# LunaJang/Metabuli_work

Hardware: AMD Instinct MI355X
Metric: reads/sec classified (150bp & 10kb) vs GTDB-scale DB at 1/2/4/8 MI355X (higher is better)
Workload: dtype u64

## Files before the change

### metabuli_work_amd/classifier.py

```python
from __future__ import annotations

import ctypes
import dataclasses
import gzip
import os
from typing import Iterator, List, Optional, Tuple

import numpy as np

from . import _abi
from ._abi import KMER_DTYPE, MATCH_DTYPE, RESULT_DTYPE, TAXCNT_DTYPE, MtbParams, ptr
from ._lib import MtbError, check, lib


@dataclasses.dataclass
class LocalParameters:
    seqMode: int = 2
    kmerFormat: int = 1
    syncmer: int = 0
    smerLen: int = 5
    reducedAA: int = 0
    skipRedundancy: int = 0
    minScore: float = 0.0
    minSpScore: float = 0.0
# ... 106 lines not shown
        return self

    def __exit__(self, *a):
        self.close()

    @property
    def db_kmers(self) -> int:
        return int(lib().mtb_db_kmers(self.handle))

    @property
    def workspace_bytes(self) -> int:
        return int(lib().mtb_workspace_bytes(self.handle))

    OPEN_PHASES = ["read_s", "decode_s", "directory_s", "probe_lines_s", "run_index_s", "taxonomy_s", "total_s",
                   "records_alloc_s"]

    def open_phases(self) -> dict:
        out = (ctypes.c_double * len(self.OPEN_PHASES))()
        lib().mtb_open_phases(self.handle, out, len(self.OPEN_PHASES))
        return {k: round(float(v), 3) for k, v in zip(self.OPEN_PHASES, out)}

    def set_workspace_cap(self, nbytes: int) -> None:
        check(lib().mtb_set_workspace_cap(self.handle, int(nbytes)), "mtb_set_workspace_cap")

    def release_workspace(self) -> None:
        self._dev_batch = None
        check(lib().mtb_release_workspace(self.handle), "mtb_release_workspace")

    def set_stream(self, stream_ptr: int) -> None:
        check(lib().mtb_set_stream(self.handle, ctypes.c_void_p(stream_ptr)), "mtb_set_stream")

    def classify_batch(self, seq1: np.ndarray, off1: np.ndarray, seq2=None, off2=None, keep_stages: bool = False,
                       device_input: bool = False, fetch: bool = True, match_only: bool = False
                       ) -> Optional[BatchResult]:
        n = (len(off1) - 1) if not device_input else int(off1.numel()) - 1
        flags = (_abi.MTB_KEEP_STAGES if keep_stages else 0) | (_abi.MTB_INPUT_DEVICE if device_input else 0)
        if match_only:
            flags |= _abi.MTB_MATCH_ONLY
            fetch = False
        if device_input:
            _after_torch(seq1)
            ptrs = [ctypes.c_void_p(t.data_ptr()) if t is not None else ctypes.c_void_p(0)
                    for t in (seq1, off1, seq2, off2)]
        else:
            ptrs = [ptr(np.ascontiguousarray(a)) if a is not None else ctypes.c_void_p(0)
                    for a in (seq1, off1, seq2, off2)]
            self._keep = (seq1, off1, seq2, off2)
        res = np.zeros(n, RESULT_DTYPE) if fetch else None
        self._dev_batch = None
        rc = check(lib().mtb_classify_batch(self.handle, ptrs[0], ptrs[1], ptrs[2], ptrs[3], n, flags,
                                            ptr(res) if fetch else ctypes.c_void_p(0)), "mtb_classify_batch")
        if rc == _abi.MTB_RETRY:
            if keep_stages or match_only or n < 2:
                raise MtbError(f"mtb_classify_batch: {lib().mtb_last_error().decode()}")
            if not fetch:
                self._classify_halves_device(seq1, off1, seq2, off2, n, device_input)
                return None
            return self._classify_halves(seq1, off1, seq2, off2, n, device_input)
        if not fetch:
            return None
        return BatchResult(res, self.taxcnt(), *self.last_counts(), self.stage_ms())

    def _classify_halves_device(self, seq1, off1, seq2, off2, n, device_input) -> None:
        import torch

        dev = torch.device("cuda", self.device)
        mid = n // 2
        recs, pools, qk, mm = [], [], 0, 0
        stats, stage, kern = None, np.zeros(5, np.float32), np.zeros(7, np.float32)
        for lo, hi in ((0, mid), (mid, n)):
            o1 = off1[lo:hi + 1]
            o2 = off2[lo:hi + 1] if off2 is not None else None
            self.classify_batch(seq1, o1, seq2, o2, device_input=device_input, fetch=False)
            rec = torch.empty((hi - lo, _abi.RESULT_DTYPE.itemsize), dtype=torch.uint8, device=dev)
            self.copy_results(rec.data_ptr(), on_device=True)
            pool = torch.empty((max(self.n_taxcnt(), 1), _abi.TAXCNT_DTYPE.itemsize), dtype=torch.uint8, device=dev)
            nt = self.copy_taxcnt(pool.data_ptr(), on_device=True)
            q, m = self.last_counts()
            recs.append(rec)
            pools.append(pool[:nt])
            qk, mm = qk + q, mm + m
            st = self.stats()
            stats = st if stats is None else {k: (max(stats[k], v) if k == "max_read_matches" else
                                                  v if k in ("join_path", "uniform_units") else stats[k] + v)
                                              for k, v in st.items()}
            stage += self.stage_ms()
            kern += self.kernel_ms()
        recs[1].view(torch.int32).view(-1, _abi.RESULT_DTYPE.itemsize // 4)[:, 4] += pools[0].shape[0]
        torch.cuda.synchronize(dev)
        self._dev_batch = _DevBatch(torch.cat(recs), torch.cat(pools), qk, mm, stats, stage, kern)

    def _classify_halves(self, seq1, off1, seq2, off2, n, device_input) -> BatchResult:
        mid = n // 2
        parts = []
        for lo, hi in ((0, mid), (mid, n)):
            o1 = off1[lo:hi + 1]
            o2 = off2[lo:hi + 1] if off2 is not None else None
            parts.append(self.classify_batch(seq1, o1, seq2, o2, device_input=device_input))
        a, b = parts
        rb = b.results.copy()
        rb["taxcnt_offset"] += len(a.taxcnt)
        return BatchResult(np.concatenate([a.results, rb]), np.concatenate([a.taxcnt, b.taxcnt]),
                           a.query_kmers + b.query_kmers, a.matches + b.matches, a.stage_ms + b.stage_ms)

    def taxcnt(self) -> np.ndarray:
        if getattr(self, "_dev_batch", None) is not None:
            return self._dev_batch.taxcnt.cpu().numpy().reshape(-1).view(TAXCNT_DTYPE).copy()
        nt = ctypes.c_uint64(0)
        lib().mtb_get_taxcnt(self.handle, ctypes.c_void_p(0), 0, ctypes.byref(nt))
        tc = np.zeros(int(nt.value), TAXCNT_DTYPE)
        check(lib().mtb_get_taxcnt(self.handle, ptr(tc), len(tc), ctypes.byref(nt)), "mtb_get_taxcnt")
        return tc

    def last_counts(self) -> Tuple[int, int]:
        if getattr(self, "_dev_batch", None) is not None:
            return self._dev_batch.query_kmers, self._dev_batch.matches
        q, m = ctypes.c_uint64(0), ctypes.c_uint64(0)
        lib().mtb_last_counts(self.handle, ctypes.byref(q), ctypes.byref(m))
        return int(q.value), int(m.value)

    STATS = ["slots", "query_kmers", "matched_queries", "matches", "max_read_matches", "groups", "groups_ge2",
             "species_runs", "wave_runs", "wave_runs_emulated", "join_path", "live_matches", "gallop_queries",
             "spilled_matches", "long_run_queries", "filter_reruns", "db_records_read", "dup_aa_queries",
             "dup_key_queries", "uniform_units"]

    def stats(self) -> dict:
        if getattr(self, "_dev_batch", None) is not None:
            return dict(self._dev_batch.stats)
        out = (ctypes.c_uint64 * len(self.STATS))()
        lib().mtb_last_stats(self.handle, out, len(self.STATS))
        return {k: int(v) for k, v in zip(self.STATS, out)}

    def stage_ms(self) -> np.ndarray:
        if getattr(self, "_dev_batch", None) is not None:
            return self._dev_batch.stage_ms.copy()
        ms = (ctypes.c_float * 5)()
        lib().mtb_last_stage_ms(self.handle, ms, 5)
        return np.array(list(ms), np.float32)

    def kernel_ms(self) -> np.ndarray:
        if getattr(self, "_dev_batch", None) is not None:
            return self._dev_batch.kernel_ms.copy()
        ms = (ctypes.c_float * 7)()
        lib().mtb_last_kernel_ms(self.handle, ms, 7)
        return np.array(list(ms), np.float32)

    def _copy_dev(self, t, dst_ptr: int, on_device: bool) -> None:
        import torch

        del on_device
        if t.numel():
            torch.cuda.synchronize(t.device)
            check(lib().mtb_memcpy(ctypes.c_void_p(dst_ptr), ctypes.c_void_p(t.data_ptr()), t.numel()), "mtb_memcpy")

    def copy_results(self, dst_ptr: int, on_device: bool = True) -> None:
        if getattr(self, "_dev_batch", None) is not None:
            return self._copy_dev(self._dev_batch.results, dst_ptr, on_device)
        check(lib().mtb_copy_results(self.handle, ctypes.c_void_p(dst_ptr), int(on_device)), "mtb_copy_results")

    def n_taxcnt(self) -> int:
        if getattr(self, "_dev_batch", None) is not None:
            return int(self._dev_batch.taxcnt.shape[0])
        nt = ctypes.c_uint64(0)
        lib().mtb_get_taxcnt(self.handle, ctypes.c_void_p(0), 0, ctypes.byref(nt))
        return int(nt.value)

    def copy_taxcnt(self, dst_ptr: int, on_device: bool = True) -> int:
        if getattr(self, "_dev_batch", None) is not None:
            self._copy_dev(self._dev_batch.taxcnt, dst_ptr, on_device)
            return int(self._dev_batch.taxcnt.shape[0])
        nt = ctypes.c_uint64(0)
        check(lib().mtb_copy_taxcnt(self.handle, ctypes.c_void_p(dst_ptr), int(on_device), ctypes.byref(nt)),
              "mtb_copy_taxcnt")
        return int(nt.value)

    def query_kmers(self) -> np.ndarray:
        q = self.stats()["query_kmers"]
        out = np.zeros(q, KMER_DTYPE)
        nq = ctypes.c_uint64(0)
        check(lib().mtb_get_query_kmers(self.handle, ptr(out), q, ctypes.byref(nq)), "mtb_get_query_kmers")
        return out

    def matches(self) -> np.ndarray:
        _, m = self.last_counts()
        out = np.zeros(m, MATCH_DTYPE)
        nm = ctypes.c_uint64(0)
        check(lib().mtb_get_matches(self.handle, ptr(out), m, ctypes.byref(nm)), "mtb_get_matches")
        return out

    def assign_matches(self, matches: np.ndarray, query_len: np.ndarray) -> BatchResult:
        matches = np.ascontiguousarray(matches, MATCH_DTYPE)
        ql = np.ascontiguousarray(query_len, np.uint32)
        res = np.zeros(len(ql), RESULT_DTYPE)
        check(lib().mtb_assign_matches(self.handle, ptr(matches), len(matches), ptr(ql), len(ql), ptr(res)),
              "mtb_assign_matches")
        return BatchResult(res, self.taxcnt(), 0, len(matches), self.stage_ms())

    def copy_matches(self, matches=None, read_counts=None, query_len=None) -> None:
        arrs = [a for a in (matches, read_counts, query_len) if a is not None]
        on_dev = bool(arrs) and not isinstance(arrs[0], np.ndarray)

        def p(a):
            if a is None:
                return ctypes.c_void_p(0)
            return ctypes.c_void_p(a.data_ptr()) if on_dev else ptr(a)
        check(lib().mtb_copy_matches(self.handle, p(matches), p(read_counts), p(query_len), int(on_dev)),
              "mtb_copy_matches")
# ... 186 lines not shown
```

### metabuli_work_amd/csrc/mtb_api.hip

```cpp
#include <chrono>
#include <cmath>
#include <cstdio>
#include <cstring>
#include <string>
#include <vector>
#include <algorithm>
#include <memory>
#include <charconv>
#include <mutex>
#include <unordered_map>

#include "mtb_host.h"
#include "mtb_launch.h"
#include <cstdlib>

using namespace mtb;

#define HIP_TRY(x)                                                                                   \
    do {                                                                                             \
        hipError_t e_ = (x);                                                                         \
        if (e_ != hipSuccess) {                                                                      \
            set_error(std::string("HIP error ") + hipGetErrorString(e_) + " at " #x);                 \
            return e_ == hipErrorOutOfMemory ? MTB_ERR_OOM : MTB_ERR_HIP;                            \
        }                                                                                            \
// ... 80 lines not shown
    uint64_t D = 0;
    DbRec* db = nullptr;
    bool borrowedDb = false;
    std::shared_ptr<DbArrays> dbArrays;
    uint64_t* dirMem = nullptr;
    ProbeLine* lines = nullptr;
    uint64_t* lineP = nullptr;
    uint16_t* runOff = nullptr;
    ProbeExt* lineExt = nullptr;
    uint64_t* link = nullptr;
    AADir dir{};
    uint64_t rankLo = 0, rankHi = ~0ull;
    int joinMode = 0;
    uint64_t* tileRec = nullptr;
    uint32_t* tilePre = nullptr;
    uint64_t nTiles = 0;
    uint32_t sweepNom = 2048;
    uint32_t sweepLdsCap = ~0u;
    bool sweepSmall = false;
    bool filterThreadMajor = false;
    int sweepPersist = 1;
    uint32_t matchWinCap = ~0u;
    bool directJoin = true;
    bool directRetry = false;
    int pruneAfter = 2;
    int bigGroups = 1;
    bool fuseFilter = true;
    bool radixDigits = true;
    bool radixAtomicFirst = false;
    int binnedSort = 0;
    uint64_t binRcForce = 0;
    bool binDigits = true;
    bool uniformUnits = true;
    uint32_t upr = 0;
    uint64_t binHost[kSortBins] = {};
    bool noFilter = false;
    uint32_t spillShift = 0;
    bool sparse = false;
    uint32_t maxW = 0;
    uint32_t maxMate = 0;
    int sortLoFine = kQuerySortLoFine;
    bool forceGeneric = false;
    bool segsortGlobal = false;
    uint32_t mergeSeg = 0;
    int waveTaxon = -1;
    int emulateAll = 0;
    bool pruneCompact = true;
    bool noAlias = false;
    uint64_t aliasBytes = 0;
    int32_t* spOf = nullptr;
    int32_t maxTax = 0;
    int32_t *tNodeOf = nullptr, *tNodeTax = nullptr, *tParent = nullptr, *tDepth = nullptr, *tSpParent = nullptr;
    uint8_t* tFlags = nullptr;
    uint32_t cladePerMatch = 2;
    std::vector<int32_t> hNodeOf;
    std::vector<std::string> hRank;
    HostTaxonomy hTax;
    mutable std::vector<std::string> lineage;
    mutable std::once_flag lineageOnce;
    std::shared_ptr<void> pipelineCache;
    mutable mtb::TaxText taxText;
    mutable std::once_flag taxTextOnce;
    WsBudget ws;
    DevBuf seq1, off1, seq2, off2, meta, reserve, slotOff, qlen, scanTmp;
    DevBuf keysA, valsA, keysB, valsB, radixCounts, radixOffs;
    DevBuf readCnt, mOff, matches, matchesSorted, segScratch, maxSeg, errFlag;
    DevBuf ordKA, ordVA, ordKB, ordVB, matchWin, unitRead, unitInfo, mStage, mRank, mTotal, mDirect, ovFlag, waveList, waveCount, devStats;
    DevBuf qFrom, probeStats;
    DevBuf longList, longCnt;
    DevBuf qStart;
    uint32_t longCap = 0;
    DevBuf chunkIn, chunkCnt, chunkSrcOff;
    DevBuf liveCnt, liveOff;
    DevBuf runFlag, runCnt, runScan;
    DevBuf segLen;
    DevBuf sizeLists;
    DevBuf digA, digB;
    DevBuf binCnt, binTab;
    DevBuf maskOut1, maskOut2, maskProb, maskScale;
    DevBuf readLens;
    DevBuf readCnt64;
    uint64_t liveM = 0;
    double openS[8] = {0, 0, 0, 0, 0, 0, 0, 0};
    static constexpr int kNumStats = 20;
    uint64_t stats[kNumStats] = {};
    uint32_t chunkC = 1;
    uint64_t stageRegion = 0;
    uint64_t spillCap = 0;
    DevBuf emMap, emCnt, emScratch, emPacked, emCnt32, emOff;
    bool emValid = false;
    bool emPackedValid = false;
    std::vector<mtb_em_map> emHost;
    std::vector<uint32_t> spKmers;
    std::string dbDir;
    DevBuf local, paths, comb, conn, spScore, spKeep,
        pathCnt, gStart, sStart, runGroup, clade, tcPool, tcLen, tcOff, tcOut, results;
    uint32_t nReads = 0;
    uint64_t Q = 0, M = 0, nTaxcnt = 0;
    uint64_t Qall = 0;
    double presentShare = 0.5;
    const uint64_t* qKeys = nullptr;
    const uint32_t* qSlots = nullptr;
    bool keepStages = false;
    bool probed = false;
    bool matchOnly = false;
    float stageMs[5] = {0, 0, 0, 0, 0};
    hipEvent_t ev[6]{};
    static constexpr int kNumKern = 7;
    float kernMs[kNumKern] = {0, 0, 0, 0, 0, 0, 0};
    hipEvent_t kev[2 * kNumKern]{};
};

static std::vector<DevBuf*> batch_bufs(mtb_ctx* c);

static void bind_workspace(mtb_ctx* c, size_t cap) {
    c->ws.cap = cap;
    if (const char* e = getenv("MTB_WORKSPACE_CAP")) {
        char* end = nullptr;
        double v = strtod(e, &end);
        const char u = end ? *end : 0;
        v *= u == 'G' || u == 'g' ? 1e9 : u == 'M' || u == 'm' ? 1e6 : u == 'K' || u == 'k' ? 1e3 : 1.0;
        c->ws.cap = v > 0 ? (size_t)v : 0;
    }
    for (DevBuf* b : batch_bufs(c)) b->budget = &c->ws;
}

static void free_db(mtb_ctx* c) {
    if (c->dbArrays) {
        c->dbArrays.reset();
        c->db = nullptr;
        c->dirMem = nullptr;
        c->lines = nullptr;
        c->lineP = nullptr;
        c->runOff = nullptr;
        c->lineExt = nullptr;
        c->link = nullptr;
        return;
    }
    if (c->borrowedDb) c->db = nullptr;
    void* ptrs[] = {c->db, c->dirMem, c->lines, c->lineP, c->runOff, c->lineExt, c->link, c->spOf, c->tNodeOf, c->tNodeTax, c->tParent, c->tDepth, c->tSpParent, c->tFlags};
    for (void* p : ptrs)
        if (p) hipFree(p);
    c->db = nullptr;
    c->dirMem = nullptr;
    c->lines = nullptr;
    c->lineP = nullptr;
    c->runOff = nullptr;
    c->lineExt = nullptr;
    c->link = nullptr;
}

template <typename T>
static hipError_t upload(T** dst, const std::vector<T>& v, hipStream_t s) {
    hipError_t e = hipMalloc((void**)dst, std::max<size_t>(1, v.size()) * sizeof(T));
    if (e != hipSuccess) return e;
    if (!v.empty()) e = hipMemcpyAsync(*dst, v.data(), v.size() * sizeof(T), hipMemcpyHostToDevice, s);
    return e;
}

static int validate_params(const mtb_params* p) {
    if (p->reduced_aa) { set_error("reduced-AA DBs (ReducedKmerMatcher) are out of scope"); return MTB_ERR_UNSUPPORTED; }
    if (p->em && p->db_parts > 1) { set_error("--em needs the whole DB in one context"); return MTB_ERR_UNSUPPORTED; }
    if (p->mask_mode && !(p->mask_prob > 0.0f && p->mask_prob <= 1.0f)) { set_error("mask_prob must be in (0, 1]"); return MTB_ERR_ARG; }
    if (p->kmer_format != 1 && p->kmer_format != 2) { set_error("kmer_format must be 1 or 2"); return MTB_ERR_UNSUPPORTED; }
    if (p->syncmer && p->kmer_format != 2) { set_error("syncmer requires kmer_format 2"); return MTB_ERR_UNSUPPORTED; }
    if (p->syncmer && (p->smer_len < 1 || p->smer_len > 8)) { set_error("smer_len must be in [1, 8]"); return MTB_ERR_ARG; }
    if (p->seq_mode < 1 || p->seq_mode > 3) { set_error("seq_mode must be 1, 2 or 3"); return MTB_ERR_ARG; }
// ... 385 lines not shown

#define MTB_BATCH_BUFS(X) \
    X(seq1) X(off1) X(seq2) X(off2) X(meta) X(reserve) X(slotOff) X(qlen) X(scanTmp) X(keysA) X(valsA) X(keysB) \
    X(valsB) X(radixCounts) X(radixOffs) X(readCnt) X(mOff) X(matches) X(matchesSorted) X(segScratch) X(maxSeg) \
    X(errFlag) X(ordKA) X(ordVA) X(ordKB) X(ordVB) X(matchWin) X(unitRead) X(unitInfo) X(waveList) X(waveCount) \
    X(devStats) X(mStage) X(mRank) X(mDirect) X(ovFlag) X(mTotal) X(qFrom) X(probeStats) X(longList) X(longCnt) \
    X(qStart) X(chunkIn) X(chunkCnt) X(chunkSrcOff) X(liveCnt) X(liveOff) X(segLen) X(sizeLists) X(digA) \
    X(digB) X(binCnt) X(binTab) X(local) X(paths) X(comb) X(conn) X(spScore) X(spKeep) X(runFlag) X(runCnt) \
    X(runScan) X(pathCnt) X(gStart) X(sStart) X(runGroup) X(clade) X(tcPool) X(tcLen) X(tcOff) X(tcOut) X(results) \
    X(emMap) X(emCnt) X(emScratch) X(emPacked) X(emCnt32) X(emOff) X(maskOut1) X(maskOut2) X(maskProb) \
    X(maskScale) X(readLens) X(readCnt64)
static std::vector<DevBuf*> batch_bufs(mtb_ctx* c) {
#define MTB_BUF_PTR(n) &c->n,
    return {MTB_BATCH_BUFS(MTB_BUF_PTR)};
#undef MTB_BUF_PTR
}

static const char* const* batch_buf_names() {
#define MTB_BUF_NAME(n) #n,
    static const char* const names[] = {MTB_BATCH_BUFS(MTB_BUF_NAME)};
#undef MTB_BUF_NAME
    return names;
}

void mtb_close(mtb_ctx* c) {
    if (!c) return;
    hipSetDevice(c->device);
    if (c->stream) hipStreamSynchronize(c->stream);
    free_db(c);
    if (c->tileRec) hipFree(c->tileRec);
    if (c->tilePre) hipFree(c->tilePre);
    c->pipelineCache.reset();
    hipSetDevice(c->device);
    for (DevBuf* b : batch_bufs(c)) b->release();
    for (auto& e : c->ev)
        if (e) hipEventDestroy(e);
    for (auto& e : c->kev)
        if (e) hipEventDestroy(e);
    if (c->ownStream && c->stream) hipStreamDestroy(c->stream);
    delete c;
}

int mtb_set_stream(mtb_ctx* c, void* stream) {
    if (!c) return MTB_ERR_ARG;
    if (c->ownStream && c->stream) hipStreamDestroy(c->stream);
    if (stream) {
        c->stream = (hipStream_t)stream;
        c->ownStream = false;
    } else {
        HIP_TRY(hipStreamCreateWithFlags(&c->stream, hipStreamNonBlocking));
        c->ownStream = true;
    }
    return MTB_OK;
}

uint64_t mtb_db_kmers(const mtb_ctx* c) { return c ? c->D : 0; }

uint64_t mtb_workspace_bytes(const mtb_ctx* c) { return c ? c->ws.used : 0; }

int mtb_open_phases(const mtb_ctx* c, double* sec, int n) {
    if (!c || !sec) return MTB_ERR_ARG;
    for (int i = 0; i < n && i < 8; i++) sec[i] = c->openS[i];
    return MTB_OK;
}

int mtb_set_workspace_cap(mtb_ctx* c, uint64_t bytes) {
    if (!c) return MTB_ERR_ARG;
    c->ws.cap = bytes;
    return MTB_OK;
}

int mtb_release_workspace(mtb_ctx* c) {
    if (!c) return MTB_ERR_ARG;
    mtb::ctx_release_workspace(c);
    void* p = nullptr;
    if (hipMalloc(&p, 64u << 20) == hipSuccess) hipFree(p);
    return hipDeviceSynchronize() == hipSuccess ? MTB_OK : MTB_ERR_HIP;
}

int mtb_ctx_device(const mtb_ctx* c) { return c ? c->device : 0; }

}

static AssignArgs assign_args(const mtb_params& p) {
    AssignArgs a;
    a.em = p.em ? 1 : 0;
    a.kmerFormat = p.kmer_format;
    if (p.syncmer) {
        a.dnaShift = (8 - p.smer_len) * 3;
        a.maxCodonShift = 8 - p.smer_len;
    } else {
        a.dnaShift = 3;
        a.maxCodonShift = 1;
    }
    a.denominator = (p.seq_mode == 1 || p.seq_mode == 2) ? 100 : 1000;
    a.minConsCnt = p.min_cons_cnt;
    a.minConsCntEuk = p.min_cons_cnt_euk;
    a.accessionLevel = p.accession_level;
    a.minScore = p.min_score;
    a.minSpScore = p.min_sp_score;
    a.tieRatio = p.tie_ratio;
    a.generic = 0;
    return a;
}

static int assign_stage(mtb_ctx* c, uint32_t n, bool keep) {
    hipStream_t s = c->stream;
    HIP_TRY(c->errFlag.ensure(sizeof(int)));
    const uint64_t M = c->M;
    AssignArgs a = assign_args(c->par);
    a.generic = c->forceGeneric ? 1 : 0;
    a.waveTaxon = c->waveTaxon;
    a.bigGroups = c->bigGroups;
    a.emulateAll = c->emulateAll;
    if (a.dnaShift <= 0) { set_error("syncmer smer_len 8 gives a zero dnaShift"); return MTB_ERR_ARG; }
    HIP_TRY(c->readCnt.ensure(sizeof(uint32_t) * (n + 1)));
    const uint64_t Mc = std::max<uint64_t>(M, 1);
    HIP_TRY(c->results.ensure(sizeof(mtb_result) * std::max<uint32_t>(n, 1)));
    HIP_TRY(c->matchesSorted.ensure(sizeof(mtb_match) * Mc));
    HIP_TRY(c->maxSeg.ensure(sizeof(uint32_t)));
    launch_max_seg(c->mOff.as<uint64_t>(), n, c->maxSeg.as<uint32_t>(), s);
    uint32_t maxSeg = 0;
    HIP_TRY(hipMemcpyAsync(&maxSeg, c->maxSeg.p, sizeof(uint32_t), hipMemcpyDeviceToHost, s));
    HIP_TRY(hipStreamSynchronize(s));
    const bool prune = !keep && !c->forceGeneric;
    if (maxSeg > kSegSortLds || c->forceGeneric || c->segsortGlobal || (c->mergeSeg && maxSeg > c->mergeSeg))
        HIP_TRY(c->segScratch.ensure(6 * sizeof(uint64_t) * Mc));
    const bool compact = prune && maxSeg > kSegSortRegs && !c->segsortGlobal && c->pruneCompact;
    if (compact) HIP_TRY(c->segLen.ensure(sizeof(uint32_t) * (n + 1)));
    if (maxSeg > 128) HIP_TRY(c->sizeLists.ensure(sizeof(uint32_t) * (4 * (size_t)n + 4)));
    c->keepStages = !prune;
    HIP_TRY(c->liveCnt.ensure(sizeof(uint32_t) * (n + 1)));
    HIP_TRY(c->liveOff.ensure(sizeof(uint64_t) * (n + 1)));
    HIP_TRY(c->scanTmp.ensure(sizeof(uint64_t) * scan_tmp_elems(n + 1)));
    HIP_TRY(hipEventRecord(c->kev[10], s));
    if (c->sparse && (!prune || (maxSeg > kSegSortSparse && !compact) || c->segsortGlobal ||
                      (c->mergeSeg && maxSeg > c->mergeSeg))) {
        launch_compact_segments(c->mDirect.as<SegMatch>(), c->slotOff.as<uint64_t>(), c->chunkC,
                                c->mOff.as<uint64_t>(), n, c->matches.as<mtb_match>(), c->spillShift, s,
                                c->stats[13] ? 2 : 0);
        c->sparse = false;
    }
    HIP_TRY(launch_segsort(c->matches.as<mtb_match>(), c->mOff.as<uint64_t>(), n, Mc, c->matchesSorted.as<mtb_match>(),
                           c->segScratch.as<uint64_t>(), maxSeg, c->forceGeneric || c->segsortGlobal,
                           prune ? c->liveCnt.as<uint32_t>() : nullptr, c->mergeSeg,
                           prune_min_matches(a.minConsCnt, a.minConsCntEuk, a.maxCodonShift), s,
                           c->sparse ? c->mDirect.as<SegMatch>() : nullptr, c->slotOff.as<uint64_t>(),
                           c->chunkC | c->spillShift << 16,
                           compact ? c->segLen.as<uint32_t>() : nullptr,
                           c->maxSeg.as<uint32_t>(), c->pruneAfter, maxSeg > 128 ? c->sizeLists.as<uint32_t>() : nullptr));
    c->sparse = false;
    const mtb_match* kIn = c->matchesSorted.as<mtb_match>();
    const uint64_t* kOff = c->mOff.as<uint64_t>();
    uint64_t kM = M;
    HIP_TRY(c->runCnt.ensure(sizeof(uint32_t) * 2 * ((size_t)n + 1)));
    HIP_TRY(c->runScan.ensure(sizeof(uint64_t) * 2 * ((size_t)n + 1)));
    uint32_t* grpCnt = c->runCnt.as<uint32_t>();
    uint32_t* runCnt = grpCnt + n + 1;
    if (prune) {
        exclusive_scan_u32(c->liveCnt.as<uint32_t>(), n, c->liveOff.as<uint64_t>(), c->scanTmp.p, s);
        HIP_TRY(hipMemcpyAsync(&kM, c->liveOff.as<uint64_t>() + n, sizeof(uint64_t), hipMemcpyDeviceToHost, s));
        HIP_TRY(hipStreamSynchronize(s));
        if (kM > M) { set_error("internal error: K5 kept more matches than it sorted"); return MTB_ERR_INTERNAL; }
        HIP_TRY(c->runFlag.ensure(std::max<uint64_t>(kM, 1)));
        launch_run_flags(c->matchesSorted.as<mtb_match>(), c->mOff.as<uint64_t>(), c->liveOff.as<uint64_t>(), n,
                         c->matches.as<mtb_match>(), c->runFlag.as<uint8_t>(), grpCnt, runCnt, c->errFlag.as<int>(),
                         s);
        kIn = c->matches.as<mtb_match>();
        kOff = c->liveOff.as<uint64_t>();
    } else {
        HIP_TRY(c->runFlag.ensure(Mc));
        launch_run_flags(kIn, kOff, kOff, n, nullptr, c->runFlag.as<uint8_t>(), grpCnt, runCnt, c->errFlag.as<int>(), s);
    }
    c->liveM = kM;
    c->stats[11] = kM;
    const uint64_t Kc = std::max<uint64_t>(kM, 1);
    const uint64_t Mn = std::max<uint64_t>(Kc, n);
    std::vector<std::pair<char*, size_t>> dead;
    if (!c->noAlias) {
        std::vector<DevBuf*> d = {&c->mDirect, &c->segScratch, &c->mStage, &c->mRank, &c->matchWin, &c->chunkIn};
        if (prune) {
            for (DevBuf* b : {&c->matchesSorted, &c->keysA, &c->valsA, &c->keysB, &c->valsB}) d.push_back(b);
        } else {
            d.push_back(&c->matches);
        }
        for (DevBuf* b : d)
            if (b->p && b->bytes >= (1u << 20)) dead.push_back({b->as<char>(), b->bytes});
        std::sort(dead.begin(), dead.end(), [](auto& a, auto& b) { return a.second > b.second; });
    }
    struct Need {
        DevBuf* own;
        uint64_t bytes;
        void* p;
    };
    Need need[] = {{&c->local, path_bytes() * Kc, nullptr},
                   {&c->paths, path_bytes() * Kc, nullptr},
                   {&c->comb, path_bytes() * Kc, nullptr},
                   {&c->conn, Kc, nullptr},
                   {&c->spScore, sizeof(float) * Kc, nullptr},
                   {&c->spKeep, Kc, nullptr},
                   {&c->waveList, sizeof(uint64_t) * Kc, nullptr},
                   {&c->pathCnt, sizeof(uint32_t) * (Kc + 1), nullptr},
                   {&c->gStart, sizeof(uint64_t) * (Kc + 1), nullptr},
                   {&c->sStart, sizeof(uint64_t) * (Kc + 1), nullptr},
                   {&c->runGroup, sizeof(uint64_t) * (Kc + 1), nullptr},
                   {&c->clade, clade_bytes() * Kc * c->cladePerMatch, nullptr},
                   {&c->tcPool, sizeof(mtb_taxcnt) * Kc, nullptr},
                   {&c->ordKA, sizeof(uint64_t) * (Mn + 1), nullptr},
                   {&c->ordVA, sizeof(uint64_t) * (Mn + 1), nullptr},
                   {&c->ordKB, sizeof(uint64_t) * (Mn + 1), nullptr},
                   {&c->ordVB, sizeof(uint64_t) * (Mn + 1), nullptr}};
    std::vector<Need*> order;
    for (Need& x : need) order.push_back(&x);
    std::stable_sort(order.begin(), order.end(), [](Need* a, Need* b) { return a->bytes > b->bytes; });
    c->aliasBytes = 0;
    for (Need* x : order) {
        const size_t b = (x->bytes + 255) & ~(size_t)255;
        for (auto& r : dead)
            if (r.second >= b) {
                x->p = r.first;
                r.first += b;
                r.second -= b;
                c->aliasBytes += b;
                break;
            }
        if (!x->p) {
            HIP_TRY(x->own->ensure(x->bytes));
            x->p = x->own->p;
        }
    }
    HIP_TRY(c->waveCount.ensure(sizeof(uint32_t)));
    HIP_TRY(hipEventRecord(c->kev[11], s));
    HIP_TRY(hipEventRecord(c->kev[12], s));
    HIP_TRY(c->radixCounts.ensure(sizeof(uint32_t) * radix_counts_elems(Mn + 1)));
    HIP_TRY(c->radixOffs.ensure(sizeof(uint64_t) * (radix_counts_elems(Mn + 1) + 1)));
    HIP_TRY(c->scanTmp.ensure(sizeof(uint64_t) * scan_tmp_elems(radix_counts_elems(Mn + 1) + n + Mn + 2)));
    TaxDevice t{c->tNodeOf, c->tNodeTax, c->tParent, c->tDepth, c->tFlags, c->tSpParent, c->maxTax};
    AssignScratch sc{need[0].p,
                     need[1].p,
                     need[2].p,
                     (uint8_t*)need[3].p,
                     (uint32_t*)need[7].p,
                     (uint64_t*)need[8].p,
                     (uint64_t*)need[9].p,
                     (uint64_t*)need[10].p,
                     c->runFlag.as<uint8_t>(),
                     grpCnt,
                     runCnt,
                     c->runScan.as<uint64_t>(),
                     c->runScan.as<uint64_t>() + n + 1,
                     (float*)need[4].p,
                     (uint64_t*)need[6].p,
                     c->waveCount.as<uint32_t>(),
                     (uint8_t*)need[5].p,
                     c->scanTmp.p,
                     (uint64_t*)need[13].p,
                     (uint64_t*)need[14].p,
                     (uint64_t*)need[15].p,
                     (uint64_t*)need[16].p,
                     c->radixCounts.as<uint32_t>(),
                     c->radixOffs.as<uint64_t>(),
                     need[11].p,
                     c->cladePerMatch};
    mtb_taxcnt* tcPool = (mtb_taxcnt*)need[12].p;
    c->stats[3] = M;
    c->stats[4] = maxSeg;
    launch_assign(kIn, kOff, c->qlen.as<uint32_t>(), n, kM, a, t, sc, tcPool,
                  c->results.as<mtb_result>(), c->devStats.as<unsigned long long>(), c->stats + 5, s);
    HIP_TRY(hipEventRecord(c->kev[13], s));
    HIP_TRY(c->tcLen.ensure(sizeof(uint32_t) * (n + 1)));
    HIP_TRY(c->tcOff.ensure(sizeof(uint64_t) * (n + 1)));
    launch_taxcnt_len(c->results.as<mtb_result>(), n, c->tcLen.as<uint32_t>(), s);
    exclusive_scan_u32(c->tcLen.as<uint32_t>(), n, c->tcOff.as<uint64_t>(), c->scanTmp.p, s);
    uint64_t NT = 0;
    HIP_TRY(hipMemcpyAsync(&NT, c->tcOff.as<uint64_t>() + n, sizeof(uint64_t), hipMemcpyDeviceToHost, s));
    HIP_TRY(hipStreamSynchronize(s));
    HIP_TRY(c->tcOut.ensure(sizeof(mtb_taxcnt) * std::max<uint64_t>(NT, 1)));
    launch_compact_taxcnt(tcPool, kOff, c->results.as<mtb_result>(), c->tcOff.as<uint64_t>(), n,
                          c->tcOut.as<mtb_taxcnt>(), s);
    c->nTaxcnt = NT;
    c->emValid = false;
    c->emPackedValid = false;
    if (c->par.em) {
        const uint64_t nS = std::max<uint64_t>(c->stats[7], 1);
        HIP_TRY(c->emScratch.ensure(8 * nS));
        HIP_TRY(c->emMap.ensure(8 * (uint64_t)kEmTop * std::max<uint32_t>(n, 1)));
        HIP_TRY(c->emCnt.ensure(std::max<uint32_t>(n, 1)));
        launch_em_top(kIn, kOff, n, sc, c->results.as<mtb_result>(), c->emScratch.p, c->emMap.p,
                      c->emCnt.as<uint8_t>(), s);
        HIP_TRY(hipGetLastError());
        c->emValid = true;
    }
    return MTB_OK;
}

static int join_stage(mtb_ctx* c, const uint8_t* dSeq1, const uint64_t* dOff1, const uint8_t* dSeq2,
                      const uint64_t* dOff2, uint32_t n, uint64_t U, uint32_t C, uint64_t R, uint64_t Rc) {
    hipStream_t s = c->stream;
    const bool probe = c->probed;
    const bool filt = c->lines && (!c->noFilter || probe);
    const bool fused = filt && !probe && c->fuseFilter;
    if (!fused) {
        HIP_TRY(c->keysA.ensure(8 * Rc));
        HIP_TRY(c->valsA.ensure(4 * Rc));
        HIP_TRY(c->keysB.ensure(8 * Rc));
        HIP_TRY(c->valsB.ensure(4 * Rc));
    }
    HIP_TRY(c->radixCounts.ensure(sizeof(uint32_t) * radix_counts_elems(Rc)));
    HIP_TRY(c->radixOffs.ensure(sizeof(uint64_t) * (radix_counts_elems(Rc) + 1)));
    HIP_TRY(c->scanTmp.ensure(sizeof(uint64_t) * scan_tmp_elems(radix_counts_elems(Rc) + n + 1)));
    HIP_TRY(c->mTotal.ensure(sizeof(unsigned long long) * kStageRegions));
    HIP_TRY(c->probeStats.ensure(sizeof(unsigned long long) * kProbeStatsLen));
    HIP_TRY(hipMemsetAsync(c->probeStats.p, 0, sizeof(unsigned long long) * kProbeStatsLen, s));
    HIP_TRY(hipEventRecord(c->kev[0], s));
    if (!fused)
        launch_extract(dSeq1, dOff1, dSeq2, dOff2, c->meta.as<ReadMeta>(), c->slotOff.as<uint64_t>(),
                       c->unitRead.as<uint32_t>(), U, C, c->tables, c->par.kmer_format, c->par.syncmer,
                       c->par.smer_len, c->keysA.as<uint64_t>(), c->unitInfo.as<uint64_t>(), s, c->upr);
    HIP_TRY(hipEventRecord(c->kev[1], s));
    uint64_t Q = R;
    const uint64_t* qk = c->keysA.as<uint64_t>();
    const uint32_t* qi = nullptr;
    const uint64_t* qf = nullptr;
    HIP_TRY(hipEventRecord(c->kev[2], s));
    const bool digits = fused && c->radixDigits && c->sortLoFine == kQuerySortLo;
    uint64_t binRc = 0;
    if (fused) {
        uint64_t cap = std::min<uint64_t>(R, (uint64_t)((double)R * c->presentShare) + 4096);
        bool binned = digits && c->binnedSort && (c->binnedSort == 2 || cap >= (1ull << 22));
        for (int pass = 0; pass < 2 && binned; pass++) {
            uint64_t rc = c->binRcForce ? c->binRcForce : (cap + cap / 16) / kSortBins + 256;
            rc = (rc + 63) / 64 * 64;
            const uint64_t slots = rc * kSortBins;
            HIP_TRY(c->keysB.ensure(8 * slots));
            HIP_TRY(c->valsB.ensure(4 * slots));
            HIP_TRY(c->digA.ensure(slots));
            HIP_TRY(c->binCnt.ensure(sizeof(unsigned long long) * kSortBins));
            Q = launch_extract_filter(dSeq1, dOff1, dSeq2, dOff2, c->meta.as<ReadMeta>(), c->slotOff.as<uint64_t>(),
                                      c->unitRead.as<uint32_t>(), U, C, c->tables, c->par.kmer_format, c->par.syncmer,
                                      c->par.smer_len, c->unitInfo.as<uint64_t>(), c->lines, c->keysB.as<uint64_t>(),
                                      c->valsB.as<uint32_t>(), c->mTotal.as<unsigned long long>(), c->rankLo,
                                      c->rankHi, &c->Qall, slots, false, s,
                                      c->binDigits ? c->digA.as<uint8_t>() : nullptr,
                                      c->binCnt.as<unsigned long long>(), rc, c->binHost, c->upr);
            HIP_TRY(hipGetLastError());
            if (R) c->presentShare = std::max(c->presentShare, std::min(1.0, 1.125 * (double)Q / (double)R));
            bool over = false;
            for (int r = 0; r < kSortBins; r++) over |= c->binHost[r] > rc;
            if (!over) {
                binRc = rc;
                break;
// ... 216 lines not shown
                    c->mRank.ensure(sizeof(uint32_t) * want) == hipSuccess) {
                    c->spillCap = want;
                    HIP_TRY(hipMemsetAsync(c->probeStats.p, 0, sizeof(unsigned long long) * kProbeStatsLen, s));
                    continue;
                }
                (void)hipGetLastError();
            }
            nSpill = 0;
            direct = false;
            if (sweep && !unstaged_join(c->lines != nullptr, c->D, Q, std::min<uint32_t>(c->matchWinCap, 3072)))
                launch_match_windows(qk, Q, c->db, c->D, c->dir, c->par.kmer_format, c->matchWin.as<uint64_t>(), s);
            HIP_TRY(c->mStage.ensure(sizeof(mtb_match) * c->stageRegion * kStageRegions));
            HIP_TRY(c->mRank.ensure(sizeof(uint32_t) * c->stageRegion * kStageRegions));
            HIP_TRY(hipMemsetAsync(c->probeStats.p, 0, sizeof(unsigned long long) * kProbeStatsLen, s));
            continue;
        }
        M = 0;
        uint64_t most = 0;
        for (unsigned long long t : regTot) {
            M += t;
            most = std::max<uint64_t>(most, t);
        }
        if (most <= c->stageRegion || M >= kMaxBatchMatches) break;
        c->stageRegion = most + most / 8;
        HIP_TRY(c->mStage.ensure(sizeof(mtb_match) * c->stageRegion * kStageRegions));
        HIP_TRY(c->mRank.ensure(sizeof(uint32_t) * c->stageRegion * kStageRegions));
        HIP_TRY(hipMemsetAsync(c->probeStats.p, 0, sizeof(unsigned long long) * kProbeStatsLen, s));
    }
    if (cnt64) launch_cnt64_counts(cnt64, n, c->readCnt.as<uint32_t>(), s);
    HIP_TRY(hipEventRecord(c->kev[7], s));
    exclusive_scan_u32(c->readCnt.as<uint32_t>(), n, c->mOff.as<uint64_t>(), c->scanTmp.p, s);
    if (direct) {
        HIP_TRY(hipMemcpyAsync(&M, c->mOff.as<uint64_t>() + n, sizeof(uint64_t), hipMemcpyDeviceToHost, s));
        HIP_TRY(hipStreamSynchronize(s));
    }
    if (M >= kMaxBatchMatches) {
        set_error("batch produced >= 2^32 matches: split it into smaller batches");
        return MTB_ERR_ARG;
    }
    c->M = M;
    HIP_TRY(c->matches.ensure(sizeof(mtb_match) * std::max<uint64_t>(M, 1)));
    HIP_TRY(hipEventRecord(c->kev[8], s));
    c->stats[13] = nSpill;
    c->sparse = direct && !c->keepStages && !c->forceGeneric && !c->matchOnly;
    if (c->sparse && nSpill) {
        launch_compact_segments(c->mDirect.as<SegMatch>(), c->slotOff.as<uint64_t>(), C, c->mOff.as<uint64_t>(), n,
                                c->matches.as<mtb_match>(), c->spillShift, s, 1);
        launch_spill_scatter(c->mStage.as<mtb_match>(), c->mRank.as<uint32_t>(), c->mTotal.as<unsigned long long>(),
                             nSpill, c->mOff.as<uint64_t>(), n, c->matches.as<mtb_match>(), c->errFlag.as<int>(), s);
    } else if (direct && !c->sparse) {
        launch_compact_segments(c->mDirect.as<SegMatch>(), c->slotOff.as<uint64_t>(), C, c->mOff.as<uint64_t>(), n,
                                c->matches.as<mtb_match>(), c->spillShift, s);
        launch_spill_scatter(c->mStage.as<mtb_match>(), c->mRank.as<uint32_t>(), c->mTotal.as<unsigned long long>(),
                             nSpill, c->mOff.as<uint64_t>(), n, c->matches.as<mtb_match>(), c->errFlag.as<int>(), s);
    } else if (!direct)
        launch_match_transpose(c->mStage.as<mtb_match>(), c->mRank.as<uint32_t>(), c->stageRegion,
                               c->mTotal.as<unsigned long long>(), c->mOff.as<uint64_t>(), n,
                               c->matches.as<mtb_match>(), c->errFlag.as<int>(), s);
    HIP_TRY(hipEventRecord(c->kev[9], s));
    HIP_TRY(hipEventRecord(c->ev[3], s));
    return MTB_OK;
}

static int batch_error(int err) {
    switch (err) {
        case kErrTaxid:
            set_error("a selected reference k-mer has taxID 0 or no species in taxID_list (KmerMatcher.cpp:432-441)");
            return MTB_ERR_DB;
        case kErrProbeStash:
            set_error("a DB AA run holds >= 2^24 k-mers (probe join stash limit): use MTB_JOIN=sort");
            return MTB_ERR_DB;
        case kErrStagedRead:
            set_error("internal error: a staged or spilled match names a read outside the batch or past its segment");
            return MTB_ERR_INTERNAL;
        case kErrProbeCount:
            set_error("internal error: emitted matches disagree with the probe counts");
            return MTB_ERR_INTERNAL;
        case kErrRunOutsideDb:
            set_error("internal error: K4 found an AA run starting past the DB's end (run index or probe lines "
                      "inconsistent with the DB records)");
            return MTB_ERR_INTERNAL;
        case kErrLiveCount:
            set_error("internal error: K5 kept more live matches than a read's segment holds");
            return MTB_ERR_INTERNAL;
        default:
            set_error("internal error: device error flag " + std::to_string(err));
            return MTB_ERR_INTERNAL;
    }
}

static int check_err_flag(mtb_ctx* c) {
    int err = 0;
    HIP_TRY(hipMemcpy(&err, c->errFlag.p, sizeof(int), hipMemcpyDeviceToHost));
    return err ? batch_error(err) : MTB_OK;
}

static int mask_mates(mtb_ctx* c, const uint8_t* seq1, const uint64_t* off1, const uint8_t* seq2, const uint64_t* off2,
                      uint32_t n, const uint8_t** out1, const uint8_t** out2) {
    hipStream_t s = c->stream;
    uint64_t nb[2] = {0, 0};
    HIP_TRY(hipMemcpyAsync(&nb[0], off1 + n, sizeof(uint64_t), hipMemcpyDeviceToHost, s));
    if (seq2) HIP_TRY(hipMemcpyAsync(&nb[1], off2 + n, sizeof(uint64_t), hipMemcpyDeviceToHost, s));
    HIP_TRY(hipStreamSynchronize(s));
    const uint64_t most = std::max(nb[0], nb[1]);
    HIP_TRY(c->maskProb.ensure(sizeof(float) * (most + 1)));
    HIP_TRY(c->maskScale.ensure(sizeof(double) * tantan_scale_elems(most, n)));
    const TantanTables tt = make_tantan_tables(c->par.mask_prob);
    HIP_TRY(c->maskOut1.ensure(nb[0] + 1));
    launch_tantan_mask(seq1, off1, n, tt, c->maskProb.as<float>(), c->maskScale.as<double>(), c->maskOut1.as<uint8_t>(), s);
    *out1 = c->maskOut1.as<uint8_t>();
    if (seq2) {
        HIP_TRY(c->maskOut2.ensure(nb[1] + 1));
        launch_tantan_mask(seq2, off2, n, tt, c->maskProb.as<float>(), c->maskScale.as<double>(),
                           c->maskOut2.as<uint8_t>(), s);
        *out2 = c->maskOut2.as<uint8_t>();
    }
    HIP_TRY(hipGetLastError());
    return MTB_OK;
}

extern "C" {

int mtb_memcpy(void* dst, const void* src, uint64_t bytes) {
    if (bytes && (!dst || !src)) { set_error("null argument"); return MTB_ERR_ARG; }
    if (bytes) HIP_TRY(hipMemcpy(dst, src, bytes, hipMemcpyDefault));
    return MTB_OK;
}

int mtb_line_ext_check(mtb_ctx* c, uint64_t* out) {
    if (!c || !out) return MTB_ERR_ARG;
    out[0] = out[1] = out[2] = 0;
    if (!c->lineExt || !c->runOff) { set_error("no run-length lines (MTB_LINE_EXT=0, or no run index)"); return MTB_ERR_ARG; }
    HIP_TRY(hipSetDevice(c->device));
    DevBuf cnt;
    HIP_TRY(cnt.ensure(3 * sizeof(unsigned long long)));
    HIP_TRY(hipMemsetAsync(cnt.p, 0, 3 * sizeof(unsigned long long), c->stream));
    launch_line_ext_check(c->lines, c->lineP, c->runOff, c->lineExt, cnt.as<unsigned long long>(), c->stream);
    HIP_TRY(hipGetLastError());
    HIP_TRY(hipMemcpyAsync(out, cnt.p, 3 * sizeof(uint64_t), hipMemcpyDeviceToHost, c->stream));
    HIP_TRY(hipStreamSynchronize(c->stream));
    if (out[2]) {
        set_error("internal error: " + std::to_string(out[2]) + " runs from the run-length lines disagree with the run index");
        return MTB_ERR_INTERNAL;
    }
    return MTB_OK;
}

int mtb_link_check(mtb_ctx* c, uint64_t* out) {
    if (!c || !out) return MTB_ERR_ARG;
    out[0] = out[1] = out[2] = 0;
    if (!c->link || !c->lines) { set_error("no link lines (MTB_LINK_LINES=0, the probe or sweep join, or no memory for them)"); return MTB_ERR_ARG; }
    HIP_TRY(hipSetDevice(c->device));
    DevBuf cnt;
    HIP_TRY(cnt.ensure(3 * sizeof(unsigned long long)));
    HIP_TRY(hipMemsetAsync(cnt.p, 0, 3 * sizeof(unsigned long long), c->stream));
    launch_link_check(c->lines, c->link, cnt.as<unsigned long long>(), c->stream);
    HIP_TRY(hipGetLastError());
    HIP_TRY(hipMemcpyAsync(out, cnt.p, 3 * sizeof(uint64_t), hipMemcpyDeviceToHost, c->stream));
    HIP_TRY(hipStreamSynchronize(c->stream));
    if (out[2]) {
        set_error("internal error: " + std::to_string(out[2]) + " link-line bits disagree with the probe lines");
        return MTB_ERR_INTERNAL;
    }
    return MTB_OK;
}

// ... 915 lines not shown
```

### metabuli_work_amd/csrc/mtb_assign.hip

```cpp
#include <algorithm>
#include <vector>

#include "mtb_launch.h"
#include "mtb_stdsort.h"

namespace mtb {

struct Path {
    int start, end;
    float score;
    int hd, depth;
    uint32_t sm, em;
};

__device__ __forceinline__ void match_key(const mtb_match& m, uint64_t& hi, uint64_t& lo) {
    hi = ((uint64_t)m.species_id << 32) | ((uint64_t)info_frame(m.qinfo) << 29) | (info_pos(m.qinfo) & 0x1FFFFFFFu);
    lo = ((uint64_t)m.hamming << 56) | ((uint64_t)(m.dna_encoding & 0xFFFFFFu) << 32) | m.target_id;
}

__device__ __forceinline__ bool key_gt(uint64_t ah, uint64_t al, uint64_t bh, uint64_t bl) {
    return ah > bh || (ah == bh && al > bl);
}

constexpr int kSmallSeg = 512;
static_assert(kSmallSeg == (int)kSegSortRegs, "one register-sort bound");
constexpr int kBlockSeg = 8192;
constexpr uint32_t kSegSkip = 0xFFFFFFFFu;

__device__ __forceinline__ long seg_len(const uint64_t* __restrict__ mOff, const uint32_t* __restrict__ segLen,
                                        uint32_t r) {
    if (!segLen) return (long)(mOff[r + 1] - mOff[r]);
    const uint32_t v = segLen[r];
    return v == kSegSkip ? -1 : (long)v;
}

template <int K, int J, int E, typename F>
__device__ __forceinline__ void bitonic_stages(F& f) {
    f(std::integral_constant<int, K>{}, std::integral_constant<int, J>{});
    if constexpr (J > 1) bitonic_stages<K, J / 2, E>(f);
    else if constexpr (K < 64 * E) bitonic_stages<K * 2, K, E>(f);
}

template <int J>
__device__ __forceinline__ uint64_t xor_lane64c(uint64_t v, int lane) {
    return (uint64_t)xor_lane<J>((uint32_t)(v >> 32), lane) << 32 | xor_lane<J>((uint32_t)v, lane);
}

template <int E>
__device__ __forceinline__ void wave_bitonic_sort(uint64_t (&h)[E], uint64_t (&l)[E], uint32_t (&x)[E], int lane) {
    auto stage = [&](auto kc, auto jc) {
        constexpr int k = decltype(kc)::value, j = decltype(jc)::value;
        if constexpr (j >= 64) {
            constexpr int js = j >> 6;
#pragma unroll
            for (int sl = 0; sl < E; sl++) {
                if (sl & js) continue;
                const int s2 = sl | js;
                const bool up = ((64 * sl + lane) & k) == 0;
                if (key_gt(h[sl], l[sl], h[s2], l[s2]) == up) {
                    const uint64_t th = h[sl], tl = l[sl];
                    const uint32_t tx = x[sl];
                    h[sl] = h[s2]; l[sl] = l[s2]; x[sl] = x[s2];
                    h[s2] = th; l[s2] = tl; x[s2] = tx;
                }
            }
        } else {
            const bool lower = (lane & j) == 0;
#pragma unroll
            for (int sl = 0; sl < E; sl++) {
                const bool up = ((64 * sl + lane) & k) == 0;
                const uint64_t ph = xor_lane64c<j>(h[sl], lane), pl = xor_lane64c<j>(l[sl], lane);
                const uint32_t px = xor_lane<j>(x[sl], lane);
                const bool takeP = (key_gt(h[sl], l[sl], ph, pl) == (lower == up));
                if (takeP) { h[sl] = ph; l[sl] = pl; x[sl] = px; }
            }
        }
    };
    bitonic_stages<2, 1, E>(stage);
}

struct MatchIn {
    const mtb_match* __restrict__ p;
    uint64_t base;
    __device__ __forceinline__ mtb_match full(uint32_t e) const { return p[base + e]; }
};
struct SegIn {
    const SegMatch* __restrict__ p;
    uint64_t base;
    uint64_t seqBits;
    __device__ __forceinline__ mtb_match full(uint32_t e) const { return seg_expand(p[base + e], seqBits); }
};

__device__ __forceinline__ bool sparse_read(const SegMatch* seg, const uint64_t* __restrict__ inOff, uint32_t inCS,
                                            uint32_t r, long n) {
    if (!seg) return false;
    const uint64_t cap = ((inOff[r + 1] - inOff[r]) * (inCS & 0xFFFFu)) >> (inCS >> 16);
    return (uint64_t)n <= cap;
}
__device__ __forceinline__ SegIn sparse_in(const SegMatch* seg, const uint64_t* __restrict__ inOff, uint32_t inCS,
                                           uint32_t r) {
    return SegIn{seg, inOff[r] * (inCS & 0xFFFFu), (uint64_t)(r + 1) << 32};
}

template <typename K>
__device__ __forceinline__ uint32_t lds_insert(K* tab, uint32_t tn, K key) {
    uint32_t i = (uint32_t)(((uint64_t)key * 0x9E3779B97F4A7C15ull) >> 40) & (tn - 1);
    while (true) {
        const K prev = atomicCAS(&tab[i], (K)0, key);
        if (prev == 0 || prev == key) return i;
        i = (i + 1) & (tn - 1);
    }
}

template <int E2>
__device__ __forceinline__ void sort_live(mtb_match* __restrict__ out, uint64_t seqBits,
                                          uint64_t base, int nLive, int lane, const uint64_t* cH,
                                          const uint64_t* cL, const uint32_t* cX) {
    uint64_t h[E2], l[E2];
    uint32_t x[E2];
#pragma unroll
    for (int sl = 0; sl < E2; sl++) {
        const int e = 64 * sl + lane;
        const bool v = e < nLive;
        h[sl] = v ? cH[e] : ~0ull;
        l[sl] = v ? cL[e] : ~0ull;
        x[sl] = v ? cX[e] : 0u;
    }
    wave_bitonic_sort<E2>(h, l, x, lane);
#pragma unroll
    for (int sl = 0; sl < E2; sl++) {
        const int e = 64 * sl + lane;
        if (e < nLive) {
            mtb_match m;
            m.qinfo = ((h[sl] >> 29) & 7ull) << 61 | seqBits | (uint32_t)(h[sl] & 0x1FFFFFFFu);
            m.target_id = (uint32_t)l[sl];
            m.species_id = (uint32_t)(h[sl] >> 32);
            m.dna_encoding = (uint32_t)(l[sl] >> 32) & 0xFFFFFFu;
            m.right_end_hamming = (uint16_t)(x[sl] >> 16);
            m.hamming = (uint8_t)(l[sl] >> 56);
            m.pad = 0;
            out[base + e] = m;
        }
    }
}

template <int E>
struct PruneLds {
    union {
        struct {
            uint32_t spKey[128 * E];
            uint32_t pairKey[128 * E];
            uint32_t pairCnt[128 * E];
        } t;
        struct {
            uint64_t cH[64 * E], cL[64 * E];
            uint32_t cX[64 * E];
        } c;
    };
};
template <int E>
__device__ __forceinline__ PruneLds<E>& prune_lds() {
    __shared__ PruneLds<E> lds;
    return lds;
}
template <int E>
__device__ __forceinline__ uint8_t* run_live_lds() {
    __shared__ uint8_t runLive[64 * E];
    return runLive;
}

template <int E, typename In>
__device__ __forceinline__ void prune_then_sort(const In& in, mtb_match* __restrict__ out, uint64_t base, int n, int lane,
                                                uint32_t* __restrict__ liveCnt, uint32_t r, uint32_t pm) {
    constexpr uint32_t T = 128 * E;
    constexpr uint32_t kLive = 0x80000000u;
    PruneLds<E>& L = prune_lds<E>();
    uint32_t *spKey = L.t.spKey, *pairKey = L.t.pairKey, *pairCnt = L.t.pairCnt;
    for (uint32_t i = lane; i < T; i += 64) {
        spKey[i] = 0;
        pairKey[i] = 0;
        pairCnt[i] = 0;
    }
    __syncthreads();
    uint64_t h[E], l[E];
    uint32_t ps[E], ss[E], rx[E];
#pragma unroll
    for (int sl = 0; sl < E; sl++) {
        const int e = 64 * sl + lane;
        h[sl] = l[sl] = 0;
        ps[sl] = ss[sl] = rx[sl] = 0;
        if (e < n) {
            const mtb_match m = in.full((uint32_t)e);
            match_key(m, h[sl], l[sl]);
            rx[sl] = (uint32_t)m.right_end_hamming << 16;
            ss[sl] = lds_insert<uint32_t>(spKey, T, (uint32_t)(h[sl] >> 32));
            ps[sl] = lds_insert<uint32_t>(pairKey, T, (ss[sl] << 3 | ((uint32_t)(h[sl] >> 29) & 7u)) + 1u);
            atomicAdd(&pairCnt[ps[sl]], 1u);
        }
    }
    __syncthreads();
#pragma unroll
    for (int sl = 0; sl < E; sl++)
        if (64 * sl + lane < n && pairCnt[ps[sl]] >= pm) spKey[ss[sl]] |= kLive;
    __syncthreads();
    bool live[E];
#pragma unroll
    for (int sl = 0; sl < E; sl++) live[sl] = 64 * sl + lane < n && (spKey[ss[sl]] & kLive);
    __syncthreads();
    uint64_t *cH = L.c.cH, *cL = L.c.cL;
    uint32_t* cX = L.c.cX;
    const uint64_t lt = (1ull << lane) - 1;
    int nLive = 0;
#pragma unroll
    for (int sl = 0; sl < E; sl++) {
        const uint64_t m = __ballot(live[sl]);
        if (live[sl]) {
            const int p = nLive + (int)__popcll(m & lt);
            cH[p] = h[sl];
            cL[p] = l[sl];
            cX[p] = rx[sl] | (uint32_t)(64 * sl + lane);
        }
        nLive += (int)__popcll(m);
    }
    __syncthreads();
    const uint64_t seqBits = nLive ? in.full(0).qinfo & (0x1FFFFFFFull << 32) : 0;
    if (nLive <= 64) sort_live<1>(out, seqBits, base, nLive, lane, cH, cL, cX);
    else if (E >= 2 && nLive <= 128) sort_live<(E >= 2 ? 2 : 1)>(out, seqBits, base, nLive, lane, cH, cL, cX);
    else if (E >= 4 && nLive <= 256) sort_live<(E >= 4 ? 4 : 1)>(out, seqBits, base, nLive, lane, cH, cL, cX);
    else sort_live<E>(out, seqBits, base, nLive, lane, cH, cL, cX);
    if (lane == 0) liveCnt[r] = (uint32_t)nLive;
}

template <int E, typename K>
__device__ __forceinline__ void wave_bitonic_keys(K (&k)[E], int lane) {
    auto stage = [&](auto kc, auto jc) {
        constexpr int kk = decltype(kc)::value, j = decltype(jc)::value;
        if constexpr (j >= 64) {
            constexpr int js = j >> 6;
#pragma unroll
            for (int sl = 0; sl < E; sl++) {
                if (sl & js) continue;
                const int s2 = sl | js;
                const bool up = ((64 * sl + lane) & kk) == 0;
                if ((k[sl] > k[s2]) == up) {
                    const K t = k[sl];
                    k[sl] = k[s2];
                    k[s2] = t;
                }
            }
        } else {
            const bool lower = (lane & j) == 0;
#pragma unroll
            for (int sl = 0; sl < E; sl++) {
                const bool up = ((64 * sl + lane) & kk) == 0;
                K pk;
                if constexpr (sizeof(K) == 8) pk = (K)xor_lane64c<j>((uint64_t)k[sl], lane);
                else pk = (K)xor_lane<j>((uint32_t)k[sl], lane);
                if ((k[sl] > pk) == (lower == up)) k[sl] = pk;
            }
        }
    };
    bitonic_stages<2, 1, E>(stage);
}

template <int ES, typename K>
__device__ __forceinline__ void lds_sort_keys(K* a, int n, int lane) {
    K k[ES];
#pragma unroll
    for (int sl = 0; sl < ES; sl++) {
        const int e = 64 * sl + lane;
        k[sl] = e < n ? a[e] : (K)~(K)0;
    }
    wave_bitonic_keys<ES, K>(k, lane);
#pragma unroll
    for (int sl = 0; sl < ES; sl++) {
        const int e = 64 * sl + lane;
        if (e < n) a[e] = k[sl];
    }
}

template <int E, typename K>
__device__ __forceinline__ void lds_sort_keys_n(K* a, int n, int lane) {
    if (n <= 64) lds_sort_keys<1, K>(a, n, lane);
    else if (E >= 2 && n <= 128) lds_sort_keys<(E >= 2 ? 2 : 1), K>(a, n, lane);
    else if (E >= 4 && n <= 256) lds_sort_keys<(E >= 4 ? 4 : 1), K>(a, n, lane);
    else lds_sort_keys<E, K>(a, n, lane);
}

template <int E>
struct RankLds {
    union {
        struct {
            uint32_t spKey[128 * E];
            uint32_t pairKey[128 * E];
            uint32_t pairCnt[128 * E];
        } t;
        struct {
            uint64_t key[64 * E];
            uint64_t lo[64 * E];
            uint32_t sp[64 * E];
            uint32_t rx[64 * E];
        } c;
    };
};

template <int E>
__device__ __forceinline__ RankLds<E>& rank_lds() {
    __shared__ RankLds<E> lds;
    return lds;
}

template <int E, typename In>
__device__ __forceinline__ void prune_rank_sort(const In& in, mtb_match* __restrict__ out, uint64_t base, int n, int lane,
                                                uint32_t* __restrict__ liveCnt, uint32_t r, uint32_t pm) {
    constexpr uint32_t T = 128 * E;
    constexpr uint32_t kLive = 0x80000000u;
    RankLds<E>& L = rank_lds<E>();
    uint32_t *spKey = L.t.spKey, *pairKey = L.t.pairKey, *pairCnt = L.t.pairCnt;
    for (uint32_t i = lane; i < T; i += 64) {
        spKey[i] = 0;
        pairKey[i] = 0;
        pairCnt[i] = 0;
    }
    __syncthreads();
    uint64_t h[E], l[E];
    uint32_t ps[E], ss[E], rx[E];
#pragma unroll
    for (int sl = 0; sl < E; sl++) {
        const int e = 64 * sl + lane;
        h[sl] = l[sl] = 0;
        ps[sl] = ss[sl] = rx[sl] = 0;
        if (e < n) {
            const mtb_match m = in.full((uint32_t)e);
            match_key(m, h[sl], l[sl]);
            rx[sl] = (uint32_t)m.right_end_hamming << 16;
            ss[sl] = lds_insert<uint32_t>(spKey, T, (uint32_t)(h[sl] >> 32));
            ps[sl] = lds_insert<uint32_t>(pairKey, T, (ss[sl] << 3 | ((uint32_t)(h[sl] >> 29) & 7u)) + 1u);
            atomicAdd(&pairCnt[ps[sl]], 1u);
        }
    }
    __syncthreads();
#pragma unroll
    for (int sl = 0; sl < E; sl++)
        if (64 * sl + lane < n && pairCnt[ps[sl]] >= pm) spKey[ss[sl]] |= kLive;
    __syncthreads();
    bool live[E];
#pragma unroll
    for (int sl = 0; sl < E; sl++) live[sl] = 64 * sl + lane < n && (spKey[ss[sl]] & kLive);
    uint32_t wide = 0;
#pragma unroll
    for (int sl = 0; sl < E; sl++) wide |= (uint32_t)(h[sl] >> 56) | ((uint32_t)(h[sl] >> 28) & 1u);
    const bool direct = __ballot(wide != 0) == 0;
    const uint64_t lt = (1ull << lane) - 1;
    if (!direct) {
        uint32_t* spList = pairCnt;
        int S = 0;
        for (uint32_t i0 = 0; i0 < T; i0 += 64) {
            const uint32_t v = spKey[i0 + lane];
            const bool lv = (v & kLive) != 0;
            const uint64_t m = __ballot(lv);
            if (lv) spList[S + (int)__popcll(m & lt)] = v & ~kLive;
            S += (int)__popcll(m);
        }
        __syncthreads();
        lds_sort_keys_n<E, uint32_t>(spList, S, lane);
        __syncthreads();
        for (int e = lane; e < S; e += 64) {
            const uint32_t v = spList[e];
            uint32_t i = (uint32_t)(((uint64_t)v * 0x9E3779B97F4A7C15ull) >> 40) & (T - 1);
            while ((spKey[i] & ~kLive) != v) i = (i + 1) & (T - 1);
            pairKey[i] = (uint32_t)e;
        }
        __syncthreads();
    }
    const int frameAt = direct ? 37 : 38;
    uint64_t key[E];
    int nLive = 0;
#pragma unroll
    for (int sl = 0; sl < E; sl++) {
        const uint64_t m = __ballot(live[sl]);
        const uint32_t p = (uint32_t)(nLive + (int)__popcll(m & lt));
        if (direct)
            key[sl] = live[sl] ? ((h[sl] >> 29) << 37 | (h[sl] & 0x0FFFFFFFull) << 9 | p) : 0;
        else
            key[sl] = live[sl] ? ((uint64_t)pairKey[ss[sl]] << 41 | ((h[sl] >> 29) & 7ull) << 38 |
                                  (h[sl] & 0x1FFFFFFFull) << 9 | p)
                               : 0;
        nLive += (int)__popcll(m);
    }
    __syncthreads();
#pragma unroll
    for (int sl = 0; sl < E; sl++)
        if (live[sl]) {
            const uint32_t p = (uint32_t)(key[sl] & 511u);
            L.c.key[p] = key[sl];
            L.c.lo[p] = l[sl];
            L.c.sp[p] = (uint32_t)(h[sl] >> 32);
            L.c.rx[p] = rx[sl];
        }
    __syncthreads();
    lds_sort_keys_n<E, uint64_t>(L.c.key, nLive, lane);
    __syncthreads();
    const uint64_t seqBits = nLive ? in.full(0).qinfo & (0x1FFFFFFFull << 32) : 0;
    for (int e = lane; e < nLive; e += 64) {
        const uint64_t k = L.c.key[e];
        const uint32_t p = (uint32_t)(k & 511u);
        const uint64_t pre = k >> 9, lo = L.c.lo[p];
        int at = e;
        for (int j = e - 1; j >= 0 && (L.c.key[j] >> 9) == pre; j--) at -= L.c.lo[L.c.key[j] & 511u] > lo;
        for (int j = e + 1; j < nLive && (L.c.key[j] >> 9) == pre; j++) at += L.c.lo[L.c.key[j] & 511u] < lo;
        mtb_match m;
        m.qinfo = ((k >> frameAt) & 7ull) << 61 | seqBits | (uint32_t)((k >> 9) & ((1ull << (frameAt - 9)) - 1));
        m.target_id = (uint32_t)lo;
        m.species_id = L.c.sp[p];
        m.dna_encoding = (uint32_t)(lo >> 32) & 0xFFFFFFu;
        m.right_end_hamming = (uint16_t)(L.c.rx[p] >> 16);
        m.hamming = (uint8_t)(lo >> 56);
        m.pad = 0;
        out[base + at] = m;
    }
    if (lane == 0) liveCnt[r] = (uint32_t)nLive;
}

template <int E, typename In>
__device__ __forceinline__ void sort_then_prune(const In& in, mtb_match* __restrict__ out, uint64_t base, int n,
                                                int lane, uint32_t* __restrict__ liveCnt, uint32_t r, uint32_t pm) {
    uint64_t h[E], l[E];
    uint32_t x[E];
#pragma unroll
    for (int sl = 0; sl < E; sl++) {
        const int e = 64 * sl + lane;
        h[sl] = ~0ull;
        l[sl] = ~0ull;
        x[sl] = 0;
        if (e < n) {
            const mtb_match m = in.full((uint32_t)e);
            match_key(m, h[sl], l[sl]);
            x[sl] = (uint32_t)m.right_end_hamming << 16;
        }
    }
    const uint64_t seqBits = in.full(0).qinfo & (0x1FFFFFFFull << 32);
    wave_bitonic_sort<E>(h, l, x, lane);
    uint8_t* runLive = run_live_lds<E>();
    const uint64_t lt = (1ull << lane) - 1;
    const int far = lane + (int)pm - 1;
    uint32_t rid[E];
    bool pair[E];
    uint32_t runs = 0;
    uint64_t prevLast = ~0ull;
#pragma unroll
    for (int sl = 0; sl < E; sl++) {
        const int e = 64 * sl + lane;
        const uint64_t sf = h[sl] >> 29;
        const uint64_t a = __shfl(sf, far & 63, 64);
        const uint64_t b = __shfl(h[sl + 1 < E ? sl + 1 : sl] >> 29, far & 63, 64);
        uint64_t pv = __shfl_up(sf, 1, 64);
        if (lane == 0) pv = prevLast;
        prevLast = __shfl(sf, 63, 64);
        pair[sl] = e + (int)pm - 1 < n && (far < 64 ? a : b) == sf;
        const bool start = e < n && (e == 0 || (pv >> 3) != (sf >> 3));
        const uint64_t m = __ballot(start);
        rid[sl] = runs + (uint32_t)__popcll(m & lt) + (uint32_t)start - 1u;
        runs += (uint32_t)__popcll(m);
        runLive[64 * sl + lane] = 0;
    }
    __syncthreads();
#pragma unroll
    for (int sl = 0; sl < E; sl++)
        if (pair[sl]) runLive[rid[sl]] = 1;
    __syncthreads();
    uint32_t kept = 0;
#pragma unroll
    for (int sl = 0; sl < E; sl++) {
        const int e = 64 * sl + lane;
        const bool live = e < n && runLive[rid[sl]];
        const uint64_t m = __ballot(live);
        if (live) {
            mtb_match o;
            o.qinfo = ((h[sl] >> 29) & 7ull) << 61 | seqBits | (uint32_t)(h[sl] & 0x1FFFFFFFu);
            o.target_id = (uint32_t)l[sl];
            o.species_id = (uint32_t)(h[sl] >> 32);
            o.dna_encoding = (uint32_t)(l[sl] >> 32) & 0xFFFFFFu;
            o.right_end_hamming = (uint16_t)(x[sl] >> 16);
            o.hamming = (uint8_t)(l[sl] >> 56);
            o.pad = 0;
            out[base + kept + (uint32_t)__popcll(m & lt)] = o;
        }
        kept += (uint32_t)__popcll(m);
    }
    if (lane == 0) liveCnt[r] = kept;
}

template <int E, typename In, int kMode = 2>
__device__ __forceinline__ void segsort_regs(const In& in, mtb_match* __restrict__ out, uint64_t base, int n, int lane,
                                             uint32_t* __restrict__ liveCnt, uint32_t r, uint32_t pm) {
    if constexpr (E >= 2 && kMode == 2) {
        if (liveCnt) {
            prune_rank_sort<E>(in, out, base, n, lane, liveCnt, r, pm);
            return;
        }
        if constexpr (E > 2) return;
    } else if constexpr (E >= 2 && kMode == 1) {
        if (liveCnt && pm <= 64) {
            sort_then_prune<E>(in, out, base, n, lane, liveCnt, r, pm);
            return;
        }
    } else if constexpr (E >= 2 && kMode == 0) {
        if (liveCnt) {
            prune_then_sort<E>(in, out, base, n, lane, liveCnt, r, pm);
            return;
        }
        if constexpr (E > 2) return;
    }
    uint64_t h[E], l[E];
    uint32_t x[E];
#pragma unroll
    for (int sl = 0; sl < E; sl++) {
        const int e = 64 * sl + lane;
        h[sl] = ~0ull;
        l[sl] = ~0ull;
        x[sl] = (uint32_t)e;
        if (e < n) match_key(in.full((uint32_t)e), h[sl], l[sl]);
    }
    wave_bitonic_sort<E>(h, l, x, lane);
    if (!liveCnt) {
#pragma unroll
        for (int sl = 0; sl < E; sl++) {
            const int e = 64 * sl + lane;
            if (e < n) out[base + e] = in.full(x[sl]);
        }
        return;
    }
    if constexpr (E == 1) {
    uint8_t* runLive = run_live_lds<E>();
    const uint64_t lt = (1ull << lane) - 1;
    bool pair[E];
    uint32_t rid[E];
    uint32_t runs = 0;
#pragma unroll
    for (int sl = 0; sl < E; sl++) {
        const int e = 64 * sl + lane;
        const uint64_t sf = h[sl] >> 29;
        const uint64_t far = __shfl(sf, min(lane + (int)pm - 1, 63), 64);
        uint64_t pv = __shfl_up(sf, 1, 64);
        if (lane == 0) pv = ~0ull;
        pair[sl] = e + (int)pm - 1 < n && far == sf;
        const bool start = e < n && (e == 0 || (pv >> 3) != (sf >> 3));
        const uint64_t m = __ballot(start);
        rid[sl] = runs + (uint32_t)__popcll(m & lt) + (uint32_t)start - 1u;
        runs += (uint32_t)__popcll(m);
        runLive[64 * sl + lane] = 0;
    }
    __syncthreads();
#pragma unroll
    for (int sl = 0; sl < E; sl++)
        if (pair[sl]) runLive[rid[sl]] = 1;
    __syncthreads();
    uint32_t kept = 0;
#pragma unroll
    for (int sl = 0; sl < E; sl++) {
        const int e = 64 * sl + lane;
        const bool live = e < n && runLive[rid[sl]];
        const uint64_t m = __ballot(live);
        if (live) out[base + kept + (uint32_t)__popcll(m & lt)] = in.full(x[sl]);
        kept += (uint32_t)__popcll(m);
    }
    if (lane == 0) liveCnt[r] = kept;
    }
}

template <typename In>
__device__ __forceinline__ void segsort_small_run(const In& in, mtb_match* __restrict__ out, uint64_t base, int n,
                                                  int lane, uint32_t* __restrict__ liveCnt, uint32_t r, uint32_t pm) {
    if (n <= 1 || (liveCnt && n < (int)pm)) {
        if (lane == 0 && n == 1 && !liveCnt) out[base] = in.full(0);
        if (lane == 0 && liveCnt) liveCnt[r] = 0;
        return;
    }
    if (n <= 64) segsort_regs<1>(in, out, base, n, lane, liveCnt, r, pm);
    else segsort_regs<2>(in, out, base, n, lane, liveCnt, r, pm);
}

__global__ void __launch_bounds__(64) k_segsort_small(const mtb_match* __restrict__ in, const uint64_t* __restrict__ mOff,
                                                      const SegMatch* __restrict__ seg,
                                                      const uint64_t* __restrict__ inOff, uint32_t inC,
                                                      uint32_t nReads, mtb_match* __restrict__ out,
                                                      uint32_t* __restrict__ liveCnt, uint32_t pm,
                                                      const uint32_t* __restrict__ segLen) {
    const uint32_t r = blockIdx.x;
    if (r >= nReads) return;
    const uint64_t base = mOff[r];
    const long nl = seg_len(mOff, segLen, r);
    if (nl < 0 || nl > 128) return;
    const int n = (int)nl;
    if (sparse_read(seg, inOff, inC, r, n)) segsort_small_run(sparse_in(seg, inOff, inC, r), out, base, n, threadIdx.x, liveCnt, r, pm);
    else segsort_small_run(MatchIn{in, base}, out, base, n, threadIdx.x, liveCnt, r, pm);
}

template <int E, int kMode>
__global__ void __launch_bounds__(64) k_segsort_regs(const mtb_match* __restrict__ in, const uint64_t* __restrict__ mOff,
                                                     const SegMatch* __restrict__ seg,
                                                     const uint64_t* __restrict__ inOff, uint32_t inC,
                                                     uint32_t nReads, mtb_match* __restrict__ out,
                                                     uint32_t* __restrict__ liveCnt, uint32_t pm,
                                                     const uint32_t* __restrict__ segLen,
                                                     const uint32_t* __restrict__ list) {
    const uint32_t r = list ? list[blockIdx.x] : blockIdx.x;
    if (r >= nReads) return;
    const uint64_t base = mOff[r];
    const long nl = seg_len(mOff, segLen, r);
    if (nl <= 32 * E || nl > 64 * E) return;
    const int n = (int)nl;
    if (sparse_read(seg, inOff, inC, r, n))
        segsort_regs<E, SegIn, kMode>(sparse_in(seg, inOff, inC, r), out, base, n,
                                       (int)threadIdx.x, liveCnt, r, pm);
    else
        segsort_regs<E, MatchIn, kMode>(MatchIn{in, base}, out, base, n, (int)threadIdx.x, liveCnt, r, pm);
}

template <int kThreads, typename Idx>
__device__ void block_bitonic(uint64_t* H, uint64_t* Lo, Idx* I, long p2) {
    for (long k = 2; k <= p2; k <<= 1)
        for (long j = k >> 1; j > 0; j >>= 1) {
            for (long t = threadIdx.x; t < (p2 >> 1); t += kThreads) {
                const long i = ((t & ~(j - 1)) << 1) | (t & (j - 1));
                const long ixj = i + j;
                const bool up = (i & k) == 0;
                const uint64_t ah = H[i], al = Lo[i], bh = H[ixj], bl = Lo[ixj];
                if (key_gt(ah, al, bh, bl) == up) {
                    H[i] = bh; Lo[i] = bl; H[ixj] = ah; Lo[ixj] = al;
                    const Idx x = I[i]; I[i] = I[ixj]; I[ixj] = x;
                }
            }
            __threadfence_block();
            __syncthreads();
        }
}

template <int kThreads>
__device__ uint32_t block_scan_u32(uint32_t x, uint32_t* total, uint32_t* sWave) {
    constexpr int kW = kThreads / 64;
    const int lane = threadIdx.x & 63, w = threadIdx.x >> 6;
    uint32_t inc = x;
#pragma unroll
    for (int d = 1; d < 64; d <<= 1) {
        const uint32_t y = __shfl_up(inc, d, 64);
        if (lane >= d) inc += y;
    }
    if (lane == 63) sWave[w] = inc;
    __syncthreads();
    if (threadIdx.x == 0) {
        uint32_t run = 0;
        for (int i = 0; i < kW; i++) {
            const uint32_t t = sWave[i];
            sWave[i] = run;
            run += t;
        }
        sWave[kW] = run;
    }
    __syncthreads();
    const uint32_t r = sWave[w] + inc - x;
    *total = sWave[kW];
    __syncthreads();
    return r;
}

template <int kThreads, typename Idx, typename In, int kSp = 32, int kSpf = 29>
__device__ uint32_t prune_pack_block(const uint64_t* H, const Idx* I, uint32_t* rid, uint8_t* runLive, long n,
                                     const In& in, mtb_match* __restrict__ out, uint64_t base,
                                     uint32_t* sWave, uint32_t pm) {
    const long per = (n + kThreads - 1) / kThreads;
    const long b = (long)threadIdx.x * per, e = min(n, b + per);
    uint32_t starts = 0;
    for (long i = b; i < e; i++) starts += (i == 0 || (H[i] >> kSp) != (H[i - 1] >> kSp)) ? 1u : 0u;
    uint32_t nRuns;
    uint32_t run = block_scan_u32<kThreads>(starts, &nRuns, sWave);
    for (long i = b; i < e; i++) {
        if (i == 0 || (H[i] >> kSp) != (H[i - 1] >> kSp)) run++;
        rid[i] = run - 1;
    }
    for (long i = threadIdx.x; i < (long)nRuns; i += kThreads) runLive[i] = 0;
    __threadfence_block();
    __syncthreads();
    for (long i = b; i < e; i++)
        if (i + (long)pm - 1 < n && (H[i] >> kSpf) == (H[i + pm - 1] >> kSpf)) runLive[rid[i]] = 1;
    __threadfence_block();
    __syncthreads();
    uint32_t mine = 0;
    for (long i = b; i < e; i++) mine += runLive[rid[i]];
    uint32_t kept;
    uint32_t at = block_scan_u32<kThreads>(mine, &kept, sWave);
    for (long i = b; i < e; i++)
        if (runLive[rid[i]]) out[base + at++] = in.full((uint32_t)I[i]);
    return kept;
}

template <int kThreads, int kPer, typename Idx, typename In>
__device__ long preprune_load(const In& in, long n, uint32_t* cnt, uint32_t* flag,
                              uint32_t logT, uint64_t* H, uint64_t* L, Idx* I, uint32_t* sWave, uint32_t pm) {
    const uint32_t T = 1u << logT;
// ... 236 lines not shown
    bool bad = false;
#pragma unroll
    for (int k = 0; k < kPer; k++) {
        h[k] = l[k] = 0;
        hp[k] = hs[k] = 0;
        if (b + k < n) {
            match_key(in.full((uint32_t)(b + k)), h[k], l[k]);
            bad |= (h[k] >> 32) >= (1ull << 24) || (h[k] & 0x1FFFFFFFull) >= (1ull << 24);
            hp[k] = (uint32_t)(((h[k] >> 29) * 0x9E3779B97F4A7C15ull) >> (64 - logT));
            hs[k] = (uint32_t)(((h[k] >> 32) * 0xC2B2AE3D27D4EB4Full) >> (64 - logT));
        }
    }
    if (__syncthreads_or(bad)) return false;
    for (uint32_t i = threadIdx.x; i < T; i += kThreads) {
        cnt[i] = 0;
        flag[i] = 0;
    }
    __syncthreads();
#pragma unroll
    for (int k = 0; k < kPer; k++)
        if (b + k < n) atomicAdd(&cnt[hp[k]], 1u);
    __syncthreads();
#pragma unroll
    for (int k = 0; k < kPer; k++)
        if (b + k < n && cnt[hp[k]] >= pm) flag[hs[k]] = 1;
    __syncthreads();
    uint32_t mask = 0;
#pragma unroll
    for (int k = 0; k < kPer; k++)
        if (b + k < n && flag[hs[k]]) mask |= 1u << k;
    uint32_t m;
    uint32_t at = block_scan_u32<kThreads>((uint32_t)__popc(mask), &m, sWave);
    if (m == 0) {
        if (threadIdx.x == 0) liveCnt[r] = 0;
        return true;
    }
#pragma unroll
    for (int k = 0; k < kPer; k++)
        if ((mask >> k) & 1u) {
            K[at] = (h[k] >> 32) << kCSp | ((h[k] >> 29) & 7ull) << kCSpf | (h[k] & 0xFFFFFFull) << kCPos | at;
            Lo[at] = l[k];
            orig[at] = (uint16_t)(b + k);
            at++;
        }
    long p2 = 2;
    while (p2 < (long)m) p2 <<= 1;
    for (long i = (long)m + threadIdx.x; i < p2; i += kThreads) K[i] = ~0ull;
    __syncthreads();
    if (bitonic) block_bitonic_u64<kThreads>(K, p2);
    else block_sort_u64<kThreads, kSeg>(K, p2);
    uint16_t pos[kPer], idx[kPer];
#pragma unroll
    for (int j = 0; j < kPer; j++) {
        const long e = threadIdx.x + (long)j * kThreads;
        pos[j] = idx[j] = 0;
        if (e < (long)m) {
            const uint64_t k = K[e], pre = k >> kCPos, lo = Lo[k & (kSeg - 1)];
            long a = e;
            for (long q = e - 1; q >= 0 && (K[q] >> kCPos) == pre; q--) a -= Lo[K[q] & (kSeg - 1)] > lo;
            for (long q = e + 1; q < (long)m && (K[q] >> kCPos) == pre; q++) a += Lo[K[q] & (kSeg - 1)] < lo;
            pos[j] = (uint16_t)a;
            idx[j] = orig[k & (kSeg - 1)];
        }
    }
    __syncthreads();
    uint16_t* placed = reinterpret_cast<uint16_t*>(Lo);
#pragma unroll
    for (int j = 0; j < kPer; j++)
        if (threadIdx.x + (long)j * kThreads < (long)m) placed[pos[j]] = idx[j];
    __syncthreads();
    uint32_t* rid = reinterpret_cast<uint32_t*>(placed + kSeg);
    const uint32_t kept = prune_pack_block<kThreads, uint16_t, In, kCSp, kCSpf>(
        K, placed, rid, reinterpret_cast<uint8_t*>(rid + kSeg), (long)m, in, out, base, sWave, pm);
    if (threadIdx.x == 0) liveCnt[r] = kept;
    return true;
}

__global__ void __launch_bounds__(kLargeThreads) k_segsort_large(const mtb_match* __restrict__ in,
                                                                 const uint64_t* __restrict__ mOff, uint32_t nReads,
                                                                 uint64_t M, mtb_match* __restrict__ out,
                                                                 uint64_t* __restrict__ gScratch, int global,
                                                                 uint32_t* __restrict__ liveCnt, long mergeSeg, uint32_t pm,
                                                                 const uint32_t* __restrict__ segLen, int compact,
                                                                 const uint32_t* __restrict__ list) {
    __shared__ uint64_t sh[kBlockSeg], sl[kBlockSeg];
    __shared__ uint16_t si[kBlockSeg];
    const uint32_t r = list ? list[blockIdx.x] : blockIdx.x;
    if (r >= nReads) return;
    const uint64_t base = mOff[r];
    long n = seg_len(mOff, segLen, r);
    if (n < 0) return;
    if (global && n == 0 && liveCnt && threadIdx.x == 0) liveCnt[r] = 0;
    if (global ? n == 0 : n <= kMidSeg) return;
    __shared__ uint32_t sWave[kLargeThreads / 64 + 1];
    long p2 = 2;
    while (p2 < n) p2 <<= 1;
    if (!global && n > mergeSeg) return;
    if (!global && liveCnt && compact &&
        segsort_compact<kLargeThreads, kBlockSeg>(MatchIn{in, base}, n, sh, sl, si, sWave, out, base, liveCnt, r, pm,
                                                  compact == 2))
        return;
    if (!global) {
        long m = n;
        if (liveCnt) {
            static_assert(kBlockSeg / kLargeThreads == 8 && 2 * kBlockSeg == 16384, "pre-prune geometry");
            m = preprune_load<kLargeThreads, 8, uint16_t>(MatchIn{in, base}, n, reinterpret_cast<uint32_t*>(sh),
                                                          reinterpret_cast<uint32_t*>(sl), 14, sh, sl, si, sWave, pm);
            if (m == 0) {
                if (threadIdx.x == 0) liveCnt[r] = 0;
                return;
            }
            p2 = 2;
            while (p2 < m) p2 <<= 1;
        }
        for (long i = threadIdx.x; i < p2; i += kLargeThreads) {
            if (liveCnt && i < m) continue;
            uint64_t h = ~0ull, l = ~0ull;
            if (i < m) match_key(in[base + i], h, l);
            sh[i] = h; sl[i] = l; si[i] = (uint16_t)i;
        }
        __syncthreads();
        block_bitonic<kLargeThreads, uint16_t>(sh, sl, si, p2);
        n = m;
        if (liveCnt) {
            uint32_t* rid = reinterpret_cast<uint32_t*>(sl);
            const uint32_t kept = prune_pack_block<kLargeThreads, uint16_t>(sh, si, rid, reinterpret_cast<uint8_t*>(rid + n),
                                                                            n, MatchIn{in, base}, out, base, sWave, pm);
            if (threadIdx.x == 0) liveCnt[r] = kept;
            return;
        }
        for (long i = threadIdx.x; i < n; i += kLargeThreads) out[base + i] = in[base + si[i]];
        return;
    }
    uint64_t* H = gScratch + 2 * base;
    uint64_t* Lo = gScratch + 2 * M + 2 * base;
    uint32_t* I = (uint32_t*)(gScratch + 4 * M) + 2 * base;
    for (long i = threadIdx.x; i < p2; i += kLargeThreads) {
        uint64_t h = ~0ull, l = ~0ull;
        if (i < n) match_key(in[base + i], h, l);
        H[i] = h; Lo[i] = l; I[i] = (uint32_t)i;
    }
    __threadfence_block();
    __syncthreads();
    block_bitonic<kLargeThreads, uint32_t>(H, Lo, I, p2);
    if (liveCnt) {
        uint32_t* rid = reinterpret_cast<uint32_t*>(Lo);
        const uint32_t kept =
            prune_pack_block<kLargeThreads, uint32_t>(H, I, rid, reinterpret_cast<uint8_t*>(rid + n), n, MatchIn{in, base},
                                                      out, base, sWave, pm);
        if (threadIdx.x == 0) liveCnt[r] = kept;
        return;
    }
    for (long i = threadIdx.x; i < n; i += kLargeThreads) out[base + i] = in[base + I[i]];
}

constexpr int kMaxPer = 8;
__device__ __forceinline__ void block_max_to(uint32_t v, uint32_t* __restrict__ out) {
    __shared__ uint32_t sM[4];
#pragma unroll
    for (int d = 32; d > 0; d >>= 1) v = max(v, (uint32_t)__shfl_xor(v, d, 64));
    if ((threadIdx.x & 63) == 0) sM[threadIdx.x >> 6] = v;
    __syncthreads();
    if (threadIdx.x == 0) {
        const uint32_t m = max(max(sM[0], sM[1]), max(sM[2], sM[3]));
        if (m) atomicMax(out, m);
    }
}
__device__ __forceinline__ uint64_t max_elem(uint32_t k) { return (uint64_t)blockIdx.x * (256 * kMaxPer) + k * 256 + threadIdx.x; }
__host__ __device__ constexpr uint32_t max_blocks(uint32_t n) { return (n + 256 * kMaxPer - 1) / (256 * kMaxPer); }

__global__ void __launch_bounds__(256) k_max_u32(const uint32_t* __restrict__ x, uint32_t n, uint32_t* __restrict__ out) {
    uint32_t v = 0;
#pragma unroll
    for (uint32_t k = 0; k < kMaxPer; k++)
        if (max_elem(k) < n) v = max(v, x[max_elem(k)]);
// ... 240 lines not shown
        const mtb_match m = in.full((uint32_t)i);
        if (cnt[pairSlot(m)] >= pm) flag[spSlot(m)] = 1;
    }
    __syncthreads();
    mtb_match* dst = inPlace ? stage : io;
    const int lane = threadIdx.x & 63;
    for (long i0 = 0; i0 < n; i0 += kLargeThreads) {
        const long i = i0 + threadIdx.x;
        const int t = (int)(i0 / kLargeThreads);
        mtb_match m;
        bool keep = false;
        if (i < n) {
            uint32_t h = 0;
#pragma unroll
            for (int x = 0; x < kThinReg; x++)
                if (x == t) h = hs2[x];
            if (t < kThinReg) {
                keep = flag[h >> 16] != 0;
                if (keep) m = in.full((uint32_t)i);
            } else {
                m = in.full((uint32_t)i);
                keep = flag[spSlot(m)] != 0;
            }
        }
        const unsigned long long mk = __ballot(keep);
        uint32_t at = 0;
        if (lane == 0 && mk) at = atomicAdd(&sCount, (uint32_t)__popcll(mk));
        at = __shfl(at, 0, 64);
        if (keep) dst[base + at + (uint32_t)__popcll(mk & ((1ull << lane) - 1))] = m;
    }
    __threadfence_block();
    __syncthreads();
    const uint32_t surv = sCount;
    if (inPlace)
        for (long i = threadIdx.x; i < (long)surv; i += kLargeThreads) io[base + i] = stage[base + i];
    if (threadIdx.x == 0) segLen[r] = surv;
}

__global__ void __launch_bounds__(256) k_max_seg_len(const uint32_t* __restrict__ segLen, uint32_t n,
                                                     uint32_t* __restrict__ out) {
    uint32_t v = 0;
#pragma unroll
    for (uint32_t k = 0; k < kMaxPer; k++)
        if (max_elem(k) < n && segLen[max_elem(k)] != kSegSkip) v = max(v, segLen[max_elem(k)]);
    block_max_to(v, out);
}

constexpr int kSizeClasses = 4;
constexpr int kSizeListReads = 1024;

__global__ void __launch_bounds__(256) k_size_lists(const uint64_t* __restrict__ mOff, const uint32_t* __restrict__ segLen,
                                                    uint32_t nReads, uint32_t maxSeg, uint32_t* __restrict__ lists,
                                                    uint32_t* __restrict__ counts) {
    __shared__ uint32_t sCnt[kSizeClasses], sBase[kSizeClasses];
    if (threadIdx.x < kSizeClasses) sCnt[threadIdx.x] = 0;
    __syncthreads();
    constexpr int kPer = kSizeListReads / 256;
    int cls[kPer];
    uint32_t at[kPer];
#pragma unroll
    for (int k = 0; k < kPer; k++) {
        const uint32_t r = blockIdx.x * kSizeListReads + k * 256 + threadIdx.x;
        cls[k] = -1;
        at[k] = 0;
        if (r < nReads) {
            const long n = seg_len(mOff, segLen, r);
            cls[k] = n > (long)maxSeg ? -1 : n > kMidSeg ? 3 : n > kSmallSeg ? 2 : n > 256 ? 1 : n > 128 ? 0 : -1;
        }
        if (cls[k] >= 0) at[k] = atomicAdd(&sCnt[cls[k]], 1u);
    }
    __syncthreads();
    if (threadIdx.x < kSizeClasses)
        sBase[threadIdx.x] = sCnt[threadIdx.x] ? atomicAdd(&counts[threadIdx.x], sCnt[threadIdx.x]) : 0u;
    __syncthreads();
#pragma unroll
    for (int k = 0; k < kPer; k++)
        if (cls[k] >= 0)
            lists[(uint64_t)cls[k] * nReads + sBase[cls[k]] + at[k]] = blockIdx.x * kSizeListReads + k * 256 + threadIdx.x;
}

static hipError_t launch_sorts(const mtb_match* in, const uint64_t* mOff, uint32_t nReads, uint64_t M, mtb_match* out,
                               uint64_t* gScratch, uint32_t maxSeg, uint32_t* liveCnt, long chunk, uint32_t pm,
                               const uint32_t* segLen, hipStream_t s, const SegMatch* seg, const uint64_t* inOff,
                               uint32_t inC, int mode, uint32_t* lists) {
    k_segsort_small<<<nReads, 64, 0, s>>>(in, mOff, seg, inOff, inC, nReads, out, liveCnt, pm, segLen);
    if (maxSeg <= 128) return hipGetLastError();
    if (!lists) {
#define MTB_REGS(E, M) k_segsort_regs<E, M><<<nReads, 64, 0, s>>>(in, mOff, seg, inOff, inC, nReads, out, liveCnt, pm, segLen, nullptr)
        if (!liveCnt) mode = 3;
        if (maxSeg > 128) {
            if (mode == 1) MTB_REGS(4, 1);
            else if (mode == 0) MTB_REGS(4, 0);
            else if (mode == 3) MTB_REGS(4, 3);
            else MTB_REGS(4, 2);
        }
        if (maxSeg > 256) {
            if (mode == 1) MTB_REGS(8, 1);
            else if (mode == 0) MTB_REGS(8, 0);
            else if (mode == 3) MTB_REGS(8, 3);
            else MTB_REGS(8, 2);
        }
#undef MTB_REGS
        if (maxSeg > kSmallSeg)
            k_segsort_mid<<<nReads, kMidThreads, 0, s>>>(in, mOff, nReads, out, liveCnt, chunk, pm, segLen, seg, inOff,
                                                         inC, mode == 2 ? 1 : mode == 4 ? 2 : 0, nullptr);
        if (maxSeg > kMidSeg)
            k_segsort_large<<<nReads, kLargeThreads, 0, s>>>(in, mOff, nReads, M, out, gScratch, 0, liveCnt, chunk, pm,
                                                             segLen, mode == 2 ? 1 : mode == 4 ? 2 : 0, nullptr);
        MTB_HIP_RET(hipGetLastError());
        if (maxSeg > chunk) return launch_merge_path(in, mOff, nReads, M, out, gScratch, liveCnt, chunk, pm, segLen, s);
        return hipSuccess;
    }
    uint32_t* dCnt = lists + (size_t)kSizeClasses * nReads;
    uint32_t cnt[kSizeClasses] = {0, 0, 0, 0};
    hipError_t e = hipMemsetAsync(dCnt, 0, sizeof(cnt), s);
    if (e == hipSuccess) {
        k_size_lists<<<(nReads + kSizeListReads - 1) / kSizeListReads, 256, 0, s>>>(mOff, segLen, nReads, maxSeg, lists, dCnt);
        e = hipGetLastError();
    }
    if (e == hipSuccess) e = hipMemcpyAsync(cnt, dCnt, sizeof(cnt), hipMemcpyDeviceToHost, s);
    if (e == hipSuccess) e = hipStreamSynchronize(s);
    const uint32_t* list4 = lists;
    const uint32_t* list8 = lists + (size_t)nReads;
    const uint32_t* listMid = lists + 2 * (size_t)nReads;
    const uint32_t* listLarge = lists + 3 * (size_t)nReads;
#define MTB_REGS(E, M, N, L) \
    k_segsort_regs<E, M><<<N, 64, 0, s>>>(in, mOff, seg, inOff, inC, nReads, out, liveCnt, pm, segLen, L)
    if (!liveCnt) mode = 3;
    if (e == hipSuccess && cnt[0]) {
        if (mode == 1) MTB_REGS(4, 1, cnt[0], list4);
        else if (mode == 0) MTB_REGS(4, 0, cnt[0], list4);
        else if (mode == 3) MTB_REGS(4, 3, cnt[0], list4);
        else MTB_REGS(4, 2, cnt[0], list4);
    }
    if (e == hipSuccess && cnt[1]) {
        if (mode == 1) MTB_REGS(8, 1, cnt[1], list8);
        else if (mode == 0) MTB_REGS(8, 0, cnt[1], list8);
        else if (mode == 3) MTB_REGS(8, 3, cnt[1], list8);
        else MTB_REGS(8, 2, cnt[1], list8);
    }
#undef MTB_REGS
    if (e == hipSuccess && cnt[2])
        k_segsort_mid<<<cnt[2], kMidThreads, 0, s>>>(in, mOff, nReads, out, liveCnt, chunk, pm, segLen, seg, inOff, inC,
                                                     mode == 2 ? 1 : mode == 4 ? 2 : 0, listMid);
    if (e == hipSuccess && cnt[3])
        k_segsort_large<<<cnt[3], kLargeThreads, 0, s>>>(in, mOff, nReads, M, out, gScratch, 0, liveCnt, chunk, pm,
                                                         segLen, mode == 2 ? 1 : mode == 4 ? 2 : 0, listLarge);
    if (e == hipSuccess) e = hipGetLastError();
    MTB_HIP_RET(e);
    if (maxSeg > chunk) return launch_merge_path(in, mOff, nReads, M, out, gScratch, liveCnt, chunk, pm, segLen, s);
    return hipSuccess;
}

hipError_t launch_segsort(const mtb_match* in, const uint64_t* mOff, uint32_t nReads, uint64_t M, mtb_match* out,
                          uint64_t* gScratch, uint32_t maxSeg, bool global, uint32_t* liveCnt, uint32_t mergeSeg,
                          uint32_t pm, hipStream_t s, const SegMatch* seg, const uint64_t* inOff, uint32_t inC,
                          uint32_t* segLen, uint32_t* maxTmp, int after, uint32_t* lists) {
    pm = max(pm, 2u);
    if (nReads == 0) return hipSuccess;
    const bool thin = liveCnt && segLen;
    if (seg && (global || (maxSeg > kSegSortSparse && !thin))) return hipErrorInvalidValue;
    const long chunk = std::max<long>(kSmallSeg, std::min<long>(mergeSeg ? mergeSeg : kBlockSeg, kBlockSeg));
    if (global) {
        k_segsort_large<<<nReads, kLargeThreads, 0, s>>>(in, mOff, nReads, M, out, gScratch, 1, liveCnt, chunk, pm,
                                                         nullptr, 0, nullptr);
        return hipGetLastError();
    }
    const long thinAbove = std::min<long>(chunk, kMidSeg);
    if (!liveCnt || maxSeg <= (uint32_t)thinAbove || !segLen)
        return launch_sorts(in, mOff, nReads, M, out, gScratch, maxSeg, liveCnt, chunk, pm, nullptr, s, seg, inOff, inC, after,
                            lists);
    MTB_HIP_RET(launch_sorts(in, mOff, nReads, M, out, gScratch, (uint32_t)thinAbove, liveCnt, chunk, pm, nullptr, s,
                             seg, inOff, inC, after, lists));
    mtb_match* io = const_cast<mtb_match*>(in);
    k_thin_big<<<nReads, kLargeThreads, 0, s>>>(io, out, mOff, nReads, thinAbove, pm, segLen, seg, inOff, inC);
    MTB_HIP_RET(hipMemsetAsync(maxTmp, 0, sizeof(uint32_t), s));
    k_max_seg_len<<<max_blocks(nReads), 256, 0, s>>>(segLen, nReads, maxTmp);
    uint32_t maxSurv = 0;
    MTB_HIP_RET(hipMemcpyAsync(&maxSurv, maxTmp, sizeof(uint32_t), hipMemcpyDeviceToHost, s));
    MTB_HIP_RET(hipStreamSynchronize(s));
    if (maxSurv == 0) return hipSuccess;
    return launch_sorts(in, mOff, nReads, M, out, gScratch, maxSurv, liveCnt, chunk, pm, segLen, s, nullptr, nullptr, 0, after,
                        lists);
}

template <bool kCopy>
__global__ void __launch_bounds__(256) k_run_flags(const mtb_match* __restrict__ in, const uint64_t* __restrict__ mOff,
                                                   const uint64_t* __restrict__ liveOff, uint32_t nReads,
                                                   mtb_match* __restrict__ out, uint8_t* __restrict__ flags,
                                                   uint32_t* __restrict__ grpCnt, uint32_t* __restrict__ runCnt,
                                                   int* __restrict__ err) {
    const uint32_t r = blockIdx.x * 4 + threadIdx.x / 64;
    const uint32_t lane = threadIdx.x & 63;
    if (r >= nReads) return;
    const uint64_t lo = liveOff[r];
    const uint64_t live = liveOff[r + 1] - lo;
    if (kCopy && (live > mOff[r + 1] - mOff[r] || liveOff[r + 1] > mOff[nReads])) {
        if (lane == 0) {
            atomicExch(err, kErrLiveCount);
            grpCnt[r] = 0;
            runCnt[r] = 0;
        }
        return;
    }
    const mtb_match* src = in + (kCopy ? mOff[r] : lo);
    uint32_t ng = 0, ns = 0;
    for (uint64_t e0 = 0; e0 < live; e0 += 64) {
        const uint64_t e = e0 + lane;
        const bool on = e < live;
        mtb_match m = {};
        if (on) m = src[e];
        const uint32_t sp = m.species_id, fr = info_frame(m.qinfo);
        uint32_t psp = __shfl_up(sp, 1, 64), pfr = __shfl_up(fr, 1, 64);
        if (lane == 0 && e0 > 0) {
            psp = src[e0 - 1].species_id;
            pfr = info_frame(src[e0 - 1].qinfo);
        }
        const bool newSp = on && (e == 0 || psp != sp);
        const bool newG = on && (newSp || pfr != fr);
        if (on) {
            if (kCopy) out[lo + e] = m;
            flags[lo + e] = (uint8_t)((uint32_t)newG | (uint32_t)newSp << 1);
        }
        ng += (uint32_t)__popcll(__ballot(newG));
        ns += (uint32_t)__popcll(__ballot(newSp));
    }
    if (lane == 0) {
        grpCnt[r] = ng;
        runCnt[r] = ns;
    }
}

void launch_run_flags(const mtb_match* in, const uint64_t* mOff, const uint64_t* liveOff, uint32_t nReads,
                      mtb_match* out, uint8_t* flags, uint32_t* grpCnt, uint32_t* runCnt, int* err, hipStream_t s) {
    if (!nReads) return;
    if (out) k_run_flags<true><<<(nReads + 3) / 4, 256, 0, s>>>(in, mOff, liveOff, nReads, out, flags, grpCnt, runCnt, err);
    else k_run_flags<false><<<(nReads + 3) / 4, 256, 0, s>>>(in, mOff, liveOff, nReads, out, flags, grpCnt, runCnt, err);
}

__global__ void __launch_bounds__(256) k_max_seg(const uint64_t* __restrict__ off, uint32_t n, uint32_t* __restrict__ out) {
    uint32_t v = 0;
#pragma unroll
    for (uint32_t k = 0; k < kMaxPer; k++)
        if (max_elem(k) < n) v = max(v, (uint32_t)min<uint64_t>(off[max_elem(k) + 1] - off[max_elem(k)], 0xFFFFFFFFull));
    block_max_to(v, out);
}

void launch_max_seg(const uint64_t* off, uint32_t n, uint32_t* out, hipStream_t s) {
    hipMemsetAsync(out, 0, sizeof(uint32_t), s);
    if (n) k_max_seg<<<max_blocks(n), 256, 0, s>>>(off, n, out);
}

void launch_max_u32(const uint32_t* x, uint32_t n, uint32_t* out, hipStream_t s) {
    hipMemsetAsync(out, 0, sizeof(uint32_t), s);
    if (n) k_max_u32<<<max_blocks(n), 256, 0, s>>>(x, n, out);
}

struct TaxView {
    const int32_t* nodeOf;
    const int32_t* nodeTax;
    const int32_t* parent;
    const int32_t* depth;
    const uint8_t* flags;
    const int32_t* spParent;
    int32_t maxTax;
    __device__ bool exists(int32_t t) const { return t >= 0 && t <= maxTax && nodeOf[t] >= 0; }
    __device__ int lca_node(int i, int j) const {
        if (i == 0 || j == 0) return 0;
        while (i != j) {
            int di = depth[i], dj = depth[j];
            if (di >= dj) i = parent[i];
            if (dj >= di) j = parent[j];
        }
        return i;
    }
    __device__ int32_t lca(int32_t a, int32_t b) const {
        if (!exists(a)) return b;
        if (!exists(b)) return a;
        return nodeTax[lca_node(nodeOf[a], nodeOf[b])];
    }
};

struct AssignCfg {
    int kmerFormat, dnaShift, maxCodonShift, denominator, minConsCnt, minConsCntEuk, accessionLevel;
    float minScore, minSpScore, tieRatio;
    int generic;
    int emulateAll;
    int em;
};

struct Clade {
    int32_t tax, parentTax;
    uint32_t count;
    int32_t removed;
};




__global__ void k_group_keys(const uint64_t* __restrict__ gStart, uint64_t nG, uint64_t* __restrict__ keys,
                             uint64_t* __restrict__ vals, uint32_t* __restrict__ pathCnt, uint32_t minGroup) {
    const uint64_t g = (uint64_t)blockIdx.x * blockDim.x + threadIdx.x;
    if (g >= nG) return;
    const uint64_t n = gStart[g + 1] - gStart[g];
    if (n < minGroup) {
        pathCnt[g] = 0;
        keys[g] = kSentinel;
    } else {
        keys[g] = g;
    }
    vals[g] = 0;
}


constexpr int kRegPos = 4;
constexpr uint64_t kBigGroup = 256;

constexpr int kAhead = 2;
template <typename R>
struct IndexCursor {
// ... 1161 lines not shown
    if (ok) {
        for (long q = gl; q <= maxQ; q += kGroupLanes) {
            const uint32_t wq = qw[g][q];
            const int32_t t = wq == 0xFFFFFFFFu ? 0 : (int32_t)(wq & 0xFFFFFFu);
            if (t == 0) continue;
            uint32_t h = ((uint32_t)t * 2654435761u) & (kGroupHash - 1);
            int probes = 0;
            while (true) {
                const int32_t prev = atomicCAS(&hk[g][h], 0, t);
                if (prev == 0 || prev == t) {
                    atomicAdd(&hc[g][h], 1u);
                    break;
                }
                h = (h + 1) & (kGroupHash - 1);
                if (++probes == kGroupHash) {
                    gFlag[g] = 1;
                    break;
                }
            }
        }
    }
    group_lds_order();
    mtb_taxcnt* tc = tcP + base;
    long nTc = -1;
    const bool packed = ok && !gFlag[g];
    if (packed) {
        static_assert(2 * kGroupHash <= kGroupQ, "the packed taxa fit the quotient table");
        long at = 0;
        for (int k0 = 0; k0 < kGroupHash; k0 += kGroupLanes) {
            const int k = k0 + gl;
            const bool v = hk[g][k] != 0;
            const uint32_t m = (uint32_t)(__ballot(v) >> gLane0) & 0xFFFFu;
            if (v) {
                const long p = at + (long)__popc(m & ((1u << gl) - 1));
                qw[g][2 * p] = (uint32_t)hk[g][k];
                qw[g][2 * p + 1] = hc[g][k];
            }
            at += (long)__popc(m);
        }
        nTc = at;
    }
    group_lds_order();
    if (packed) {
        for (long e = gl; e < nTc; e += kGroupLanes) {
            const int32_t t = (int32_t)qw[g][2 * e];
            long at = 0;
            for (long j = 0; j < nTc; j++) at += (int32_t)qw[g][2 * j] < t;
            tc[at].tax_id = t;
            tc[at].count = qw[g][2 * e + 1];
        }
    }
    if (gl != 0 || !valid) return;
    if (!filter) {
        res.score = spTotal;
        if (isLCA && n > 0 && !(spTotal == 0 || spTotal < cfg.minScore)) {
            res.is_classified = 1;
            res.classification = bestTax;
        }
        results[r] = res;
        return;
    }
    if (nTc < 0) nTc = filter_redundant_serial(M, bestFirst, bestSecond, runGroup[bestRun], gStart, dnaShift, tax, tc);
    classify_tail(res, tc, nTc, spTotal, bestTax, readLength, cfg, tax, cladeP + base * cladePerMatch,
                  n * (long)cladePerMatch);
    results[r] = res;
}

__global__ void k_wave_size_keys(const uint64_t* __restrict__ waveList, uint32_t n, uint64_t* __restrict__ keys) {
    const uint32_t i = blockIdx.x * blockDim.x + threadIdx.x;
    if (i < n) keys[i] = (uint64_t)(kWaveCombineMax - (uint32_t)(waveList[i] >> 32));
}
__global__ void k_read_size_keys(const uint64_t* __restrict__ mOff, uint32_t n, uint64_t* __restrict__ keys) {
    const uint32_t i = blockIdx.x * blockDim.x + threadIdx.x;
    if (i < n) keys[i] = 0xFFFFFFull - min<uint64_t>(mOff[i + 1] - mOff[i], 0xFFFFFFull);
}

static const uint64_t* longest_first(uint32_t n, int bits, const AssignScratch& s, hipStream_t st) {
    bool inB = false;
    radix_sort_pairs(s.ordKA, s.ordVA, s.ordKB, s.ordVB, n, 0, bits, false, true, s.radixCounts, s.radixOffs,
                     s.scanTmp, &inB, st);
    return inB ? s.ordVB : s.ordVA;
}

void launch_assign(const mtb_match* matches, const uint64_t* mOff, const uint32_t* qlen, uint32_t nReads, uint64_t nM, const AssignArgs& a, const TaxDevice& t, const AssignScratch& s,
                   mtb_taxcnt* tcPool, mtb_result* results, unsigned long long* devStats, uint64_t* hostStats,
                   hipStream_t st) {
    for (int i = 0; i < 4; i++) hostStats[i] = 0;
    if (nReads == 0) return;
    AssignCfg cfg{a.kmerFormat, a.dnaShift, a.maxCodonShift, a.denominator, a.minConsCnt, a.minConsCntEuk,
                  a.accessionLevel, a.minScore, a.minSpScore, a.tieRatio, a.generic, a.emulateAll, a.em};
    TaxView tv{t.nodeOf, t.nodeTax, t.parent, t.depth, t.flags, t.spParent, t.maxTax};
    exclusive_scan_u32(s.grpCnt, nReads, s.grpOff, s.scanTmp, st);
    exclusive_scan_u32(s.runCnt, nReads, s.runOff, s.scanTmp, st);
    if (nM) {
        launch_run_starts(s.runFlag, mOff, s.grpOff, s.runOff, nReads, s.gStart, s.sStart, s.runGroup, st);
        uint64_t cnt[2] = {0, 0};
        hipMemcpyAsync(&cnt[0], s.grpOff + nReads, sizeof(uint64_t), hipMemcpyDeviceToHost, st);
        hipMemcpyAsync(&cnt[1], s.runOff + nReads, sizeof(uint64_t), hipMemcpyDeviceToHost, st);
        hipStreamSynchronize(st);
        hostStats[0] = cnt[0];
        hostStats[2] = cnt[1];
        if (cnt[0]) {
            k_group_keys<<<(unsigned)((cnt[0] + 255) / 256), 256, 0, st>>>(
                s.gStart, cnt[0], s.ordKA, s.ordVA, s.pathCnt,
                prune_min_matches(a.minConsCnt, a.minConsCntEuk, a.maxCodonShift));
            bool inB = false;
            const uint64_t heavy = radix_sort_pairs(s.ordKA, s.ordVA, s.ordKB, s.ordVB, cnt[0], 32, 40, true, false,
                                                    s.radixCounts, s.radixOffs, s.scanTmp, &inB, st);
            hostStats[1] = heavy;
            if (heavy) {
                const bool waves = !a.generic && a.bigGroups && nM >= kBigGroup;
                if (waves) hipMemsetAsync(s.waveCount, 0, sizeof(uint32_t), st);
                const char* nl = getenv("MTB_PATHS_NOLDS");
                const bool noLds = nl && atoi(nl) == 4;
                const char* la = getenv("MTB_K6_LOOKAHEAD");
                const bool look = !la || atoi(la) != 0;
#define MTB_PATHS(L, W, A)                                                                                          \
    k_match_paths<L, W, A><<<(unsigned)((heavy + 63) / 64), 64, 0, st>>>(                                              \
        matches, s.gStart, inB ? s.ordKB : s.ordKA, heavy, cfg, tv, (Path*)s.local, (Path*)s.paths, s.conn,         \
        s.pathCnt, waves ? s.waveList : nullptr, s.waveCount)
                if (noLds && look) MTB_PATHS(false, 4, true);
                else if (noLds) MTB_PATHS(false, 4, false);
                else if (look) MTB_PATHS(true, 1, true);
                else MTB_PATHS(true, 1, false);
#undef MTB_PATHS
                if (waves) {
                    uint32_t nBig = 0;
                    hipMemcpyAsync(&nBig, s.waveCount, sizeof(uint32_t), hipMemcpyDeviceToHost, st);
                    hipStreamSynchronize(st);
                    if (nBig && look)
                        k_match_paths_wave<true><<<nBig, 64, 0, st>>>(matches, s.gStart, s.waveList, cfg, tv, (Path*)s.local,
                                                                      (Path*)s.paths, s.conn, s.pathCnt);
                    else if (nBig)
                        k_match_paths_wave<false><<<nBig, 64, 0, st>>>(matches, s.gStart, s.waveList, cfg, tv, (Path*)s.local,
                                                                       (Path*)s.paths, s.conn, s.pathCnt);
                }
            }
        }
        if (cnt[1]) {
            hipMemsetAsync(s.waveCount, 0, sizeof(uint32_t), st);
            k_combine_paths<<<(unsigned)((cnt[1] + 255) / 256), 256, 0, st>>>(
                matches, s.sStart, cnt[1], s.runGroup, s.gStart, s.pathCnt, qlen, cfg, (Path*)s.paths, (Path*)s.comb,
                s.spScore, s.spKeep, s.waveList, s.waveCount);
            uint32_t nWave = 0;
            hipMemcpyAsync(&nWave, s.waveCount, sizeof(uint32_t), hipMemcpyDeviceToHost, st);
            hipStreamSynchronize(st);
            if (nWave) {
                k_wave_size_keys<<<(nWave + 255) / 256, 256, 0, st>>>(s.waveList, nWave, s.ordKA);
                const uint64_t* order = longest_first(nWave, 16, s, st);
                k_combine_wave<<<nWave, 64, 0, st>>>(matches, s.sStart, s.waveList, qlen, cfg, (Path*)s.paths,
                                                     (Path*)s.comb, s.spScore, s.spKeep, devStats, order);
            }
            hostStats[3] = nWave;
        }
    }
    const bool wave = a.waveTaxon >= 0 ? a.waveTaxon == 1 : (!a.generic && nM > (uint64_t)kWavePerReadMatches * nReads);
    const bool group = a.waveTaxon == 2 || (a.waveTaxon < 0 && !wave && !a.generic);
    if (group) {
        k_choose_taxon_group<<<(nReads + 15) / 16, 256, 0, st>>>(matches, mOff, qlen, nReads, s.runOff, s.sStart,
                                                                 s.runGroup, s.gStart, s.spScore, s.spKeep, cfg, tv,
                                                                 (Clade*)s.clade, s.cladePerMatch, tcPool, results);
    } else if (wave) {
        k_read_size_keys<<<(nReads + 255) / 256, 256, 0, st>>>(mOff, nReads, s.ordKA);
        const uint64_t* order = longest_first(nReads, 24, s, st);
        k_choose_taxon_wave<<<nReads, 64, 0, st>>>(matches, mOff, qlen, nReads, s.runOff, s.sStart, s.runGroup, s.gStart,
                                                   s.spScore, s.spKeep, cfg, tv, (Clade*)s.clade, s.cladePerMatch,
                                                   tcPool, results, order);
    } else {
        const unsigned ctT = nReads < 256u * 256u ? 64u : 256u;
        k_choose_taxon<<<(nReads + ctT - 1) / ctT, ctT, 0, st>>>(matches, mOff, qlen, nReads, s.runOff, s.sStart,
                                                             s.runGroup, s.gStart, s.spScore, s.spKeep, cfg, tv,
                                                             (Clade*)s.clade, s.cladePerMatch, tcPool, results);
    }
}

uint64_t path_bytes() { return sizeof(Path); }
uint64_t clade_bytes() { return sizeof(Clade); }

__global__ void k_compact_taxcnt(const mtb_taxcnt* __restrict__ pool, const uint64_t* __restrict__ mOff,
                                 mtb_result* __restrict__ results, const uint64_t* __restrict__ tcOff, uint32_t nReads,
                                 mtb_taxcnt* __restrict__ out) {
    uint32_t r = blockIdx.x * blockDim.x + threadIdx.x;
    if (r >= nReads) return;
    uint32_t len = results[r].taxcnt_len;
    uint64_t dst = tcOff[r];
    results[r].taxcnt_offset = (uint32_t)dst;
    for (uint32_t k = 0; k < len; k++) out[dst + k] = pool[mOff[r] + k];
}

__global__ void k_taxcnt_len(const mtb_result* __restrict__ results, uint32_t nReads, uint32_t* __restrict__ len) {
    uint32_t r = blockIdx.x * blockDim.x + threadIdx.x;
    if (r < nReads) len[r] = results[r].taxcnt_len;
}

void launch_taxcnt_len(const mtb_result* results, uint32_t nReads, uint32_t* len, hipStream_t s) {
    if (nReads) k_taxcnt_len<<<(nReads + 255) / 256, 256, 0, s>>>(results, nReads, len);
}
void launch_compact_taxcnt(const mtb_taxcnt* pool, const uint64_t* mOff, mtb_result* results, const uint64_t* tcOff,
                           uint32_t nReads, mtb_taxcnt* out, hipStream_t s) {
    if (nReads) k_compact_taxcnt<<<(nReads + 255) / 256, 256, 0, s>>>(pool, mOff, results, tcOff, nReads, out);
}

__global__ void k_chunk_totals(const uint32_t* __restrict__ cnt, uint32_t nChunks, uint32_t n,
                               uint32_t* __restrict__ tot) {
    const uint32_t r = blockIdx.x * blockDim.x + threadIdx.x;
    if (r >= n) return;
    uint32_t t = 0;
    for (uint32_t c = 0; c < nChunks; c++) t += cnt[(uint64_t)c * n + r];
    tot[r] = t;
}

__global__ void __launch_bounds__(256) k_regroup_chunks(const uint64_t* __restrict__ src, const uint32_t* __restrict__ cnt,
                                                        const uint64_t* __restrict__ srcOff, uint32_t nChunks, uint32_t n,
                                                        const uint64_t* __restrict__ mOff, uint64_t* __restrict__ dst) {
    const uint32_t r = blockIdx.x * 4 + threadIdx.x / 64;
    const uint32_t lane = threadIdx.x & 63;
    if (r >= n) return;
    uint64_t at = mOff[r] * 3;
    for (uint32_t c = 0; c < nChunks; c++) {
        const uint64_t k = (uint64_t)c * n + r;
        const uint64_t words = (uint64_t)cnt[k] * 3, from = srcOff[k] * 3;
        for (uint64_t w = lane; w < words; w += 64) dst[at + w] = src[from + w];
        at += words;
    }
}

void launch_regroup_chunks(const mtb_match* src, const uint32_t* cnt, uint32_t nChunks, uint32_t n, uint32_t* tot,
                           uint64_t* srcOff, uint64_t* mOff, void* scanTmp, mtb_match* dst, hipStream_t s) {
    if (!n) return;
    k_chunk_totals<<<(n + 255) / 256, 256, 0, s>>>(cnt, nChunks, n, tot);
    exclusive_scan_u32(tot, n, mOff, scanTmp, s);
    exclusive_scan_u32(cnt, (uint64_t)nChunks * n, srcOff, scanTmp, s);
    k_regroup_chunks<<<(n + 3) / 4, 256, 0, s>>>((const uint64_t*)src, cnt, srcOff, nChunks, n, mOff, (uint64_t*)dst);
}

struct EmPair {
    int32_t sp;
    float sc;
};

__global__ void k_em_top(const mtb_match* __restrict__ M, const uint64_t* __restrict__ mOff, uint32_t n,
                         const uint64_t* __restrict__ runOff, const uint64_t* __restrict__ sStart,
                         const float* __restrict__ spScore, const uint8_t* __restrict__ spKeep,
                         const mtb_result* __restrict__ results, EmPair* __restrict__ scratch,
                         EmPair* __restrict__ maps, uint8_t* __restrict__ cnt) {
    const uint32_t r = blockIdx.x * blockDim.x + threadIdx.x;
    if (r >= n) return;
    cnt[r] = 0;
    if (!results[r].is_classified) return;
    const uint64_t s0 = runOff[r], s1 = runOff[r + 1];
    EmPair* v = scratch + s0;
    long k = 0;
    for (uint64_t s = s0; s < s1; s++)
        if (spKeep[s]) v[k++] = EmPair{(int32_t)M[sStart[s]].species_id, spScore[s]};
    stdsort::sort(v, v + k, [](const EmPair& a, const EmPair& b) { return a.sc > b.sc; });
    const long m = k < kEmTop ? k : kEmTop;
// ... 203 lines not shown
```

### metabuli_work_amd/csrc/mtb_launch.h

```cpp
#pragma once
#include <hip/hip_runtime.h>
#include <stdint.h>

#include <utility>

#include "mtb_device.h"

namespace mtb {

constexpr int kErrTaxid = 1;
constexpr int kErrStagedRead = 2;
constexpr int kErrProbeStash = 3;
constexpr int kErrProbeCount = 4;
constexpr int kErrRunOutsideDb = 5;
constexpr int kErrLiveCount = 6;

struct ReadMeta {
    int32_t len1, len2, ql1, ql2, w1, w2;
};

struct HostTables {
    uint8_t base[256];
    int8_t aa[64];
    int8_t num[64];
};

struct TaxDevice {
    const int32_t* nodeOf;
    const int32_t* nodeTax;
    const int32_t* parent;
    const int32_t* depth;
    const uint8_t* flags;
    const int32_t* spParent;
    int32_t maxTax;
};

struct AssignArgs {
    int kmerFormat, dnaShift, maxCodonShift, denominator, minConsCnt, minConsCntEuk, accessionLevel;
    float minScore, minSpScore, tieRatio;
    int generic;
    int waveTaxon = -1;
    int emulateAll = 0;
    int em = 0;
    int bigGroups = 1;
};

struct AssignScratch {
    void* local;
    void* paths;
    void* comb;
    uint8_t* conn;
    uint32_t* pathCnt;
    uint64_t *gStart, *sStart;
    uint64_t* runGroup;
    const uint8_t* runFlag;
    const uint32_t *grpCnt, *runCnt;
    uint64_t *grpOff, *runOff;
    float* spScore;
    uint64_t* waveList;
    uint32_t* waveCount;
    uint8_t* spKeep;
    void* scanTmp;
    uint64_t *ordKA, *ordVA, *ordKB, *ordVB;
    uint32_t* radixCounts;
    uint64_t* radixOffs;
    void* clade;
    uint32_t cladePerMatch;
};

uint64_t scan_tmp_elems(uint64_t n);
inline unsigned stride_grid(uint64_t n, unsigned block = 256) {
    const uint64_t b = (n + block - 1) / block;
    return (unsigned)(b < 1 ? 1 : (b > (1ull << 22) ? (1ull << 22) : b));
}
#define MTB_GRID_STRIDE(i, n) \
    for (uint64_t i = (uint64_t)blockIdx.x * blockDim.x + threadIdx.x; i < (n); i += (uint64_t)gridDim.x * blockDim.x)
void exclusive_scan_u32(const uint32_t* in, uint64_t n, uint64_t* out, void* tmp, hipStream_t s);
void exclusive_scan_u64(const uint64_t* in, uint64_t n, uint64_t* out, void* tmp, hipStream_t s);
void exclusive_scan_u32_out32(const uint32_t* in, uint64_t n, uint32_t* out, void* tmp, hipStream_t s);
void launch_run_starts(const uint8_t* flags, const uint64_t* mOff, const uint64_t* grpOff, const uint64_t* runOff,
                       uint32_t nReads, uint64_t* gStart, uint64_t* sStart, uint64_t* runGroup, hipStream_t s);

constexpr uint32_t kSeqStage = 10240;
constexpr uint32_t kSeqMate = 219;
static_assert(23 * 2 * kSeqMate <= kSeqStage && 44 * kSeqMate <= kSeqStage, "a uniform block's bases fit the stage");
void launch_read_meta(const uint64_t* off1, const uint64_t* off2, uint32_t n, int paired, ReadMeta* meta,
                      uint32_t* qlen, uint32_t* maxW, uint32_t* readLens, hipStream_t s);
void launch_read_units(const ReadMeta* meta, uint32_t n, uint32_t C, uint32_t upr, uint32_t* units, hipStream_t s);
void launch_unit_read(const uint64_t* uOff, uint32_t n, uint32_t* unitRead, hipStream_t s);
uint64_t extract_slots(uint64_t nUnits, uint32_t C);
void launch_extract(const uint8_t* seq1, const uint64_t* off1, const uint8_t* seq2, const uint64_t* off2,
                    const ReadMeta* meta, const uint64_t* uOff, const uint32_t* unitRead, uint64_t nUnits,
                    uint32_t C, const HostTables& t, int kmerFormat, int syncmer, int smerLen, uint64_t* keys,
                    uint64_t* unitInfo, hipStream_t s, uint32_t upr = 0);

uint64_t radix_counts_elems(uint64_t n);
template <typename V>
uint64_t radix_sort_pairs(uint64_t* keysA, V* valsA, uint64_t* keysB, V* valsB, uint64_t n, int bitLo, int bitHi,
                          bool filter, bool genVals, uint32_t* counts, uint64_t* offs, void* scanTmp, bool* inB,
                          hipStream_t s, uint8_t* digA = nullptr, uint8_t* digB = nullptr, bool unstableFirst = false);
constexpr int kSortBins = 2048;
uint64_t radix_binned_tiles(const uint64_t* binHost, uint64_t rc);
template <typename V>
uint64_t radix_sort_binned(uint64_t* keysR, V* valsR, uint64_t* keysT, V* valsT, const uint64_t* binHost,
                           const unsigned long long* binDev, uint64_t rc, int bitLo, int bitHi, uint32_t* counts,
                           uint64_t* offs, void* scanTmp, uint64_t* tileTab, bool* inT, hipStream_t s, uint8_t* digR,
                           uint8_t* digT);
void launch_to_rank_form(uint64_t* v, uint64_t n, hipStream_t s);
uint64_t host_from_rank_form(uint64_t v);
constexpr uint64_t kAARankEnd = 37822859361ull;
constexpr int kQuerySortLo = 36, kQuerySortHi = 60;
constexpr int kQuerySortLoFine = 36;

uint64_t decode_diff_chunk(const uint16_t* diff, uint64_t n, uint64_t carry, uint64_t* values, uint32_t* flagTmp,
                           uint64_t* idxTmp, void* scanTmp, uint64_t* lastTerm, uint64_t* lastValue, hipStream_t s);
void launch_mask_info(uint32_t* info, uint64_t n, uint32_t mask, hipStream_t s);

struct DbRec {
    uint32_t lo, hi, tax;
};
static_assert(sizeof(DbRec) == 12, "12-B DB records");
void launch_pack_db(const uint64_t* v, const uint32_t* tax, uint64_t n, DbRec* out, hipStream_t s);
void launch_rec_rank_form(DbRec* db, uint64_t n, hipStream_t s);
void launch_rec_mask_info(DbRec* db, uint64_t n, uint32_t mask, hipStream_t s);

struct AADir {
    const uint64_t* dir;
    uint64_t R;
    uint64_t div;
    int L;
    int fmt;
};
AADir make_aa_dir(uint64_t D, int kmerFormat);
void build_aa_dir(const DbRec* db, uint64_t D, const AADir& d, uint64_t* dir, hipStream_t s);

constexpr uint32_t kLineRanks = 448;
struct alignas(64) ProbeLine {
    uint64_t base;
    uint32_t bits[kLineRanks / 32];
};
// ... 42 lines not shown
                  mtb_match* buf, uint32_t* bufRank, uint64_t region, int* err, unsigned long long* stats,
                  hipStream_t s);

constexpr uint32_t kSegMaxTax = (1u << 24) - 1;
struct SegMatch {
    uint32_t posFrame, targetHam, speciesReh, dnaReh;
};
static_assert(sizeof(SegMatch) == 16, "16-B segment matches");
__host__ __device__ inline SegMatch seg_pack(const mtb_match& m) {
    return SegMatch{(uint32_t)m.qinfo | (uint32_t)(m.qinfo >> 61) << 29, m.target_id | (uint32_t)m.hamming << 24,
                    m.species_id | (uint32_t)(m.right_end_hamming & 0xFFu) << 24,
                    (m.dna_encoding & 0xFFFFFFu) | (uint32_t)(m.right_end_hamming >> 8) << 24};
}
__host__ __device__ inline mtb_match seg_expand(const SegMatch& s, uint64_t seqBits) {
    mtb_match m;
    m.qinfo = (uint64_t)(s.posFrame >> 29) << 61 | seqBits | (s.posFrame & 0x1FFFFFFFu);
    m.target_id = s.targetHam & 0xFFFFFFu;
    m.species_id = s.speciesReh & 0xFFFFFFu;
    m.dna_encoding = s.dnaReh & 0xFFFFFFu;
    m.right_end_hamming = (uint16_t)((s.speciesReh >> 24) | (s.dnaReh >> 24) << 8);
    m.hamming = (uint8_t)(s.targetHam >> 24);
    m.pad = 0;
    return m;
}

constexpr uint32_t kStageRegions = 256;
struct LongRun {
    uint64_t q;
    uint64_t lo, hi;
};
void launch_match_long(const LongRun* list, uint32_t n, const uint64_t* qkey, const uint32_t* qslot,
                       const uint64_t* unitInfo, uint32_t C, const DbRec* db, uint64_t D, const int32_t* spOf,
                       uint32_t maxTax, int kmerFormat, uint32_t* readCnt, unsigned long long* total, mtb_match* buf,
                       uint32_t* bufRank, uint64_t region, int* err, SegMatch* direct, const uint64_t* dirOff,
                       int* overflow, uint32_t capShift, unsigned long long* stats, hipStream_t s, unsigned long long* cnt64 = nullptr);
uint64_t sweep_tiles(uint64_t D, uint32_t nom);
constexpr uint64_t kSweepStarts = (1ull << 24) + 1;
constexpr uint64_t kSweepStartsTmp = kSweepStarts + (kSweepStarts + 1023) / 1024;
void build_sweep_tiles(const DbRec* db, uint64_t D, uint32_t nom, uint64_t* pstartTmp, uint64_t* tileRec,
                       uint32_t* tilePre, hipStream_t s);
void build_query_starts(const uint64_t* qkey, uint64_t Q, uint32_t* qStart, const uint32_t* tilePre, uint64_t nTiles,
                        uint32_t* tileQ, hipStream_t s);
void launch_sweep(const uint64_t* tileRec, const uint32_t* tileQ, uint64_t nTiles, const uint64_t* qkey,
                  const uint32_t* qslot, const uint64_t* unitInfo, uint32_t C, const DbRec* db, uint64_t D,
                  const int32_t* spOf, uint32_t maxTax, int kmerFormat, uint32_t* readCnt, unsigned long long* total,
                  mtb_match* buf, uint32_t* bufRank, uint64_t region, int* err, unsigned long long* stats,
                  SegMatch* direct, int* overflow, uint32_t capShift, LongRun* longList, uint32_t longCap,
                  uint32_t* longCnt, uint32_t ldsCap, bool small, int persist, hipStream_t s);
void launch_match(const uint64_t* qkey, const uint32_t* qslot, const uint64_t* unitInfo, uint32_t C, uint64_t Q,
                  const DbRec* db, uint64_t D, const AADir& dir, const int32_t* spOf,
                  uint32_t maxTax, int kmerFormat, uint32_t* readCnt, unsigned long long* total, mtb_match* buf,
                  uint32_t* bufRank, uint64_t region, int* err, uint32_t winCap, const uint64_t* win,
                  const ProbeLine* lines, const uint64_t* lineP, const uint16_t* runOff, int sortLo,
                  unsigned long long* stats, SegMatch* direct, const uint64_t* dirOff, int* overflow,
                  uint32_t capShift, LongRun* longList, uint32_t longCap, uint32_t* longCnt, hipStream_t s,
                  const ProbeExt* lineExt = nullptr, uint32_t upr = 0, unsigned long long* cnt64 = nullptr);
void launch_cnt64_init(const uint32_t* readLens, uint32_t n, unsigned long long* cnt64, hipStream_t s);
void launch_cnt64_counts(const unsigned long long* cnt64, uint32_t n, uint32_t* readCnt, hipStream_t s);
void launch_compact_segments(const SegMatch* in, const uint64_t* dirOff, uint32_t C, const uint64_t* readOff,
                             uint32_t nReads, mtb_match* out, uint32_t capShift, hipStream_t s, int mode = 0);
void launch_spill_scatter(const mtb_match* spill, const uint32_t* spillRank, const unsigned long long* total,
                          uint64_t nSpill, const uint64_t* readOff, uint32_t nReads, mtb_match* out, int* err,
                          hipStream_t s);
bool unstaged_join(bool lines, uint64_t D, uint64_t Q, uint32_t winCap);
void launch_match_transpose(const mtb_match* buf, const uint32_t* bufRank, uint64_t region,
                            const unsigned long long* total, const uint64_t* readOff, uint32_t nReads, mtb_match* out,
                            int* err, hipStream_t s);
uint64_t match_window_elems(uint64_t Q);
void launch_dup_stats(const uint64_t* qkey, uint64_t Q, unsigned long long* out, hipStream_t s);
void launch_hamming_check(const uint64_t* a, const uint64_t* b, uint64_t n, uint8_t* sum, uint16_t* fwd, uint16_t* rev,
                          unsigned long long* bad, hipStream_t s);
void launch_pin_eval(int fn, const int64_t* param, const uint64_t* a, const uint64_t* b, uint64_t n, int64_t* out,
                     hipStream_t s);
void launch_match_windows(const uint64_t* qkey, uint64_t Q, const DbRec* db, uint64_t D, const AADir& dir,
                          int kmerFormat, uint64_t* win, hipStream_t s);

uint64_t path_bytes();
uint64_t clade_bytes();
hipError_t launch_segsort(const mtb_match* in, const uint64_t* mOff, uint32_t nReads, uint64_t M, mtb_match* out,
                          uint64_t* gScratch, uint32_t maxSeg, bool global, uint32_t* liveCnt, uint32_t mergeSeg,
                          uint32_t pruneMin, hipStream_t s, const SegMatch* seg = nullptr,
                          const uint64_t* inOff = nullptr, uint32_t inC = 0 ,
                          uint32_t* segLen = nullptr,
                          uint32_t* maxTmp = nullptr, int pruneAfter = 0, uint32_t* lists = nullptr);
inline uint32_t prune_min_matches(int minConsCnt, int minConsCntEuk, int maxCodonShift) {
    const int d = minConsCnt < minConsCntEuk ? minConsCnt : minConsCntEuk;
    const int sh = maxCodonShift > 0 ? maxCodonShift : 1;
    const int need = d <= 1 ? 1 : 1 + (d - 1 + sh - 1) / sh;
    return (uint32_t)(need < 2 ? 2 : need);
}
void launch_run_flags(const mtb_match* in, const uint64_t* mOff, const uint64_t* liveOff, uint32_t nReads,
                      mtb_match* out, uint8_t* flags, uint32_t* grpCnt, uint32_t* runCnt, int* err, hipStream_t s);
void launch_max_u32(const uint32_t* x, uint32_t n, uint32_t* out, hipStream_t s);
void launch_max_seg(const uint64_t* off, uint32_t n, uint32_t* out, hipStream_t s);
constexpr uint32_t kSegSortLds = 8192;
constexpr uint32_t kSegSortRegs = 512;
constexpr uint32_t kSegSortSparse = 2048;
constexpr uint64_t kMaxBatchMatches = 0xFFFFFFFFull;
void launch_assign(const mtb_match* matches, const uint64_t* mOff, const uint32_t* qlen, uint32_t nReads, uint64_t nM, const AssignArgs& a, const TaxDevice& t, const AssignScratch& s,
                   mtb_taxcnt* tcPool, mtb_result* results, unsigned long long* devStats, uint64_t* hostStats,
                   hipStream_t st);
void launch_regroup_chunks(const mtb_match* src, const uint32_t* cnt, uint32_t nChunks, uint32_t n, uint32_t* tot,
                           uint64_t* srcOff, uint64_t* mOff, void* scanTmp, mtb_match* dst, hipStream_t s);
void launch_taxcnt_len(const mtb_result* results, uint32_t nReads, uint32_t* len, hipStream_t s);
void launch_compact_taxcnt(const mtb_taxcnt* pool, const uint64_t* mOff, mtb_result* results, const uint64_t* tcOff,
                           uint32_t nReads, mtb_taxcnt* out, hipStream_t s);

constexpr int kEmTop = 10;
void launch_em_top(const mtb_match* M, const uint64_t* mOff, uint32_t n, const AssignScratch& s,
                   const mtb_result* results, void* scratch, void* maps, uint8_t* cnt, hipStream_t st);
void launch_em_pack(const void* maps, const uint8_t* cnt, uint32_t n, uint32_t* cnt32, uint64_t* off, void* scanTmp,
                    mtb_em_map* out, hipStream_t s);
void launch_species_kmers(const DbRec* db, uint64_t D, const int32_t* spOf, uint32_t maxTax, uint32_t* cnt,
                          hipStream_t s);
void launch_em_iteration(const float* score, const uint32_t* spIdx, const uint64_t* qOff, uint64_t nQ,
                         const uint64_t* pos, const double* p, const double* lf, double* wS,
                         unsigned long long* qCount, const uint64_t* sliceOff, uint64_t nSl, double* part,
                         const uint64_t* spSlice, uint32_t S, const uint8_t* isTop, double* pNew, double* absd,
                         int afterTen, double* delta, hipStream_t s);
void launch_em_reclassify(const float* score, const uint32_t* spIdx, const int32_t* spTax, const uint64_t* qOff,
                          const uint32_t* qId, uint64_t nQ, const double* p, const double* lf, const TaxDevice& t,
                          mtb_em_read* out, hipStream_t s);

struct HostTaxonomy;
constexpr uint64_t kSplitByUnique = ~0ull;
int encode_sorted_kmers(const uint64_t* keys, const uint64_t* pay, uint64_t kept, const HostTaxonomy& T, int splitNum,
                        uint64_t splitTotal, bool deviceOut, int kmerFormat, void* scanTmp, hipEvent_t evDedupe,
                        hipStream_t s, mtb_db_built* out);
constexpr uint32_t kMergeDbPer = 8;
constexpr uint32_t kMergeDbTile = 256 * kMergeDbPer;

constexpr int kTantanOffsets = 50;
struct TantanTables {
    double lr[25];
    double b2f[kTantanOffsets];
    double b2b, f2b, f2f;
    double minMask;
};
TantanTables make_tantan_tables(float maskProb);
uint64_t tantan_scale_elems(uint64_t bases, uint32_t n);
void launch_tantan_mask(const uint8_t* seq, const uint64_t* off, uint32_t n, const TantanTables& tt, float* prob,
                        double* scale, uint8_t* out, hipStream_t s);

}
```

Measured before the change: 34.63 million.

## Count group and species runs in K5 sort and build run index directly

The segmented sort/prune kernel (K5) now counts per-read groups and species runs with wave ballots as it sorts. The host scans these counts early, and a new pack kernel writes gStart/sStart/runGroup directly while compacting live matches. This removes the run-flag byte array pass and the separate run_starts kernel with its scans, and it sizes those index buffers by the actual group and run totals. In exchange it adds ballot work inside the sort kernels, two extra scans and host readbacks before the existing sync, and a consistency check with a new error code.

```diff
diff --git a/metabuli_work_amd/classifier.py b/metabuli_work_amd/classifier.py
--- a/metabuli_work_amd/classifier.py
+++ b/metabuli_work_amd/classifier.py
@@ -212,7 +212,7 @@
             qk, mm = qk + q, mm + m
             st = self.stats()
             stats = st if stats is None else {k: (max(stats[k], v) if k == "max_read_matches" else
-                                                  v if k in ("join_path", "uniform_units") else stats[k] + v)
+                                                  v if k in ("join_path", "uniform_units", "k6_index") else stats[k] + v)
                                               for k, v in st.items()}
             stage += self.stage_ms()
             kern += self.kernel_ms()
@@ -252,7 +252,7 @@
     STATS = ["slots", "query_kmers", "matched_queries", "matches", "max_read_matches", "groups", "groups_ge2",
              "species_runs", "wave_runs", "wave_runs_emulated", "join_path", "live_matches", "gallop_queries",
              "spilled_matches", "long_run_queries", "filter_reruns", "db_records_read", "dup_aa_queries",
-             "dup_key_queries", "uniform_units"]
+             "dup_key_queries", "uniform_units", "k6_index"]
 
     def stats(self) -> dict:
         if getattr(self, "_dev_batch", None) is not None:
diff --git a/metabuli_work_amd/csrc/mtb_api.hip b/metabuli_work_amd/csrc/mtb_api.hip
--- a/metabuli_work_amd/csrc/mtb_api.hip
+++ b/metabuli_work_amd/csrc/mtb_api.hip
@@ -186,7 +186,7 @@
     DevBuf readCnt64;
     uint64_t liveM = 0;
     double openS[8] = {0, 0, 0, 0, 0, 0, 0, 0};
-    static constexpr int kNumStats = 20;
+    static constexpr int kNumStats = 21;
     uint64_t stats[kNumStats] = {};
     uint32_t chunkC = 1;
     uint64_t stageRegion = 0;
@@ -738,6 +738,8 @@
 
 }
 
+static int batch_error(int err);
+
 static AssignArgs assign_args(const mtb_params& p) {
     AssignArgs a;
     a.em = p.em ? 1 : 0;
@@ -797,6 +799,13 @@
                                 c->stats[13] ? 2 : 0);
         c->sparse = false;
     }
+    HIP_TRY(c->runCnt.ensure(sizeof(uint32_t) * 2 * ((size_t)n + 1)));
+    HIP_TRY(c->runScan.ensure(sizeof(uint64_t) * 2 * ((size_t)n + 1)));
+    uint32_t* grpCnt = c->runCnt.as<uint32_t>();
+    uint32_t* runCnt = grpCnt + n + 1;
+    uint64_t* grpOff = c->runScan.as<uint64_t>();
+    uint64_t* runOff = grpOff + n + 1;
+    bool counted = false;
     HIP_TRY(launch_segsort(c->matches.as<mtb_match>(), c->mOff.as<uint64_t>(), n, Mc, c->matchesSorted.as<mtb_match>(),
                            c->segScratch.as<uint64_t>(), maxSeg, c->forceGeneric || c->segsortGlobal,
                            prune ? c->liveCnt.as<uint32_t>() : nullptr, c->mergeSeg,
@@ -804,32 +813,37 @@
                            c->sparse ? c->mDirect.as<SegMatch>() : nullptr, c->slotOff.as<uint64_t>(),
                            c->chunkC | c->spillShift << 16,
                            compact ? c->segLen.as<uint32_t>() : nullptr,
-                           c->maxSeg.as<uint32_t>(), c->pruneAfter, maxSeg > 128 ? c->sizeLists.as<uint32_t>() : nullptr));
+                           c->maxSeg.as<uint32_t>(), c->pruneAfter, maxSeg > 128 ? c->sizeLists.as<uint32_t>() : nullptr,
+                           prune ? grpCnt : nullptr, &counted));
     c->sparse = false;
     const mtb_match* kIn = c->matchesSorted.as<mtb_match>();
     const uint64_t* kOff = c->mOff.as<uint64_t>();
     uint64_t kM = M;
-    HIP_TRY(c->runCnt.ensure(sizeof(uint32_t) * 2 * ((size_t)n + 1)));
-    HIP_TRY(c->runScan.ensure(sizeof(uint64_t) * 2 * ((size_t)n + 1)));
-    uint32_t* grpCnt = c->runCnt.as<uint32_t>();
-    uint32_t* runCnt = grpCnt + n + 1;
+    const char* ki = getenv("MTB_K6_INDEX");
+    const bool index = prune && counted && !(ki && !strcmp(ki, "flags"));
+    uint64_t idxTot[2] = {kM, kM};
     if (prune) {
         exclusive_scan_u32(c->liveCnt.as<uint32_t>(), n, c->liveOff.as<uint64_t>(), c->scanTmp.p, s);
+        if (index) {
+            exclusive_scan_u32(grpCnt, n, grpOff, c->scanTmp.p, s);
+            exclusive_scan_u32(runCnt, n, runOff, c->scanTmp.p, s);
+            HIP_TRY(hipMemcpyAsync(&idxTot[0], grpOff + n, sizeof(uint64_t), hipMemcpyDeviceToHost, s));
+            HIP_TRY(hipMemcpyAsync(&idxTot[1], runOff + n, sizeof(uint64_t), hipMemcpyDeviceToHost, s));
+        }
         HIP_TRY(hipMemcpyAsync(&kM, c->liveOff.as<uint64_t>() + n, sizeof(uint64_t), hipMemcpyDeviceToHost, s));
         HIP_TRY(hipStreamSynchronize(s));
         if (kM > M) { set_error("internal error: K5 kept more matches than it sorted"); return MTB_ERR_INTERNAL; }
-        HIP_TRY(c->runFlag.ensure(std::max<uint64_t>(kM, 1)));
-        launch_run_flags(c->matchesSorted.as<mtb_match>(), c->mOff.as<uint64_t>(), c->liveOff.as<uint64_t>(), n,
-                         c->matches.as<mtb_match>(), c->runFlag.as<uint8_t>(), grpCnt, runCnt, c->errFlag.as<int>(),
-                         s);
+        if (index && (idxTot[0] > kM || idxTot[1] > idxTot[0])) {
+            set_error("internal error: K5 counted more groups than live matches, or more species runs than groups");
+            return MTB_ERR_INTERNAL;
+        }
+        if (!index) idxTot[0] = idxTot[1] = kM;
         kIn = c->matches.as<mtb_match>();
         kOff = c->liveOff.as<uint64_t>();
-    } else {
-        HIP_TRY(c->runFlag.ensure(Mc));
-        launch_run_flags(kIn, kOff, kOff, n, nullptr, c->runFlag.as<uint8_t>(), grpCnt, runCnt, c->errFlag.as<int>(), s);
     }
     c->liveM = kM;
     c->stats[11] = kM;
+    c->stats[20] = index ? 1 : 0;
     const uint64_t Kc = std::max<uint64_t>(kM, 1);
     const uint64_t Mn = std::max<uint64_t>(Kc, n);
     std::vector<std::pair<char*, size_t>> dead;
@@ -844,10 +858,14 @@
             if (b->p && b->bytes >= (1u << 20)) dead.push_back({b->as<char>(), b->bytes});
         std::sort(dead.begin(), dead.end(), [](auto& a, auto& b) { return a.second > b.second; });
     }
+    const uint64_t Gc = std::max<uint64_t>(idxTot[0], 1), Sc = std::max<uint64_t>(idxTot[1], 1);
+    const char* packIn = index ? c->matchesSorted.as<char>() : nullptr;
+    const size_t packInBytes = index ? c->matchesSorted.bytes : 0;
     struct Need {
         DevBuf* own;
         uint64_t bytes;
         void* p;
+        bool early = false;
     };
     Need need[] = {{&c->local, path_bytes() * Kc, nullptr},
                    {&c->paths, path_bytes() * Kc, nullptr},
@@ -857,9 +875,9 @@
                    {&c->spKeep, Kc, nullptr},
                    {&c->waveList, sizeof(uint64_t) * Kc, nullptr},
                    {&c->pathCnt, sizeof(uint32_t) * (Kc + 1), nullptr},
-                   {&c->gStart, sizeof(uint64_t) * (Kc + 1), nullptr},
-                   {&c->sStart, sizeof(uint64_t) * (Kc + 1), nullptr},
-                   {&c->runGroup, sizeof(uint64_t) * (Kc + 1), nullptr},
+                   {&c->gStart, sizeof(uint64_t) * (Gc + 1), nullptr, index},
+                   {&c->sStart, sizeof(uint64_t) * (Sc + 1), nullptr, index},
+                   {&c->runGroup, sizeof(uint64_t) * (Sc + 1), nullptr, index},
                    {&c->clade, clade_bytes() * Kc * c->cladePerMatch, nullptr},
                    {&c->tcPool, sizeof(mtb_taxcnt) * Kc, nullptr},
                    {&c->ordKA, sizeof(uint64_t) * (Mn + 1), nullptr},
@@ -873,7 +891,7 @@
     for (Need* x : order) {
         const size_t b = (x->bytes + 255) & ~(size_t)255;
         for (auto& r : dead)
-            if (r.second >= b) {
+            if (r.second >= b && !(x->early && r.first >= packIn && r.first < packIn + packInBytes)) {
                 x->p = r.first;
                 r.first += b;
                 r.second -= b;
@@ -884,6 +902,18 @@
             HIP_TRY(x->own->ensure(x->bytes));
             x->p = x->own->p;
         }
+    }
+    if (index) {
+        launch_pack_index(c->matchesSorted.as<mtb_match>(), c->mOff.as<uint64_t>(), c->liveOff.as<uint64_t>(), n,
+                          c->matches.as<mtb_match>(), grpOff, runOff, (uint64_t*)need[8].p, (uint64_t*)need[9].p,
+                          (uint64_t*)need[10].p, c->errFlag.as<int>(), s);
+    } else if (prune) {
+        HIP_TRY(c->runFlag.ensure(std::max<uint64_t>(kM, 1)));
+        launch_run_flags(c->matchesSorted.as<mtb_match>(), c->mOff.as<uint64_t>(), c->liveOff.as<uint64_t>(), n,
+                         c->matches.as<mtb_match>(), c->runFlag.as<uint8_t>(), grpCnt, runCnt, c->errFlag.as<int>(), s);
+    } else {
+        HIP_TRY(c->runFlag.ensure(Mc));
+        launch_run_flags(kIn, kOff, kOff, n, nullptr, c->runFlag.as<uint8_t>(), grpCnt, runCnt, c->errFlag.as<int>(), s);
     }
     HIP_TRY(c->waveCount.ensure(sizeof(uint32_t)));
     HIP_TRY(hipEventRecord(c->kev[11], s));
@@ -903,8 +933,12 @@
                      c->runFlag.as<uint8_t>(),
                      grpCnt,
                      runCnt,
-                     c->runScan.as<uint64_t>(),
-                     c->runScan.as<uint64_t>() + n + 1,
+                     grpOff,
+                     runOff,
+                     index,
+                     c->errFlag.as<int>(),
+                     index ? idxTot[0] : 0,
+                     index ? idxTot[1] : 0,
                      (float*)need[4].p,
                      (uint64_t*)need[6].p,
                      c->waveCount.as<uint32_t>(),
@@ -921,8 +955,9 @@
     mtb_taxcnt* tcPool = (mtb_taxcnt*)need[12].p;
     c->stats[3] = M;
     c->stats[4] = maxSeg;
-    launch_assign(kIn, kOff, c->qlen.as<uint32_t>(), n, kM, a, t, sc, tcPool,
-                  c->results.as<mtb_result>(), c->devStats.as<unsigned long long>(), c->stats + 5, s);
+    if (const int derr = launch_assign(kIn, kOff, c->qlen.as<uint32_t>(), n, kM, a, t, sc, tcPool, c->results.as<mtb_result>(),
+                                       c->devStats.as<unsigned long long>(), c->stats + 5, s))
+        return batch_error(derr);
     HIP_TRY(hipEventRecord(c->kev[13], s));
     HIP_TRY(c->tcLen.ensure(sizeof(uint32_t) * (n + 1)));
     HIP_TRY(c->tcOff.ensure(sizeof(uint64_t) * (n + 1)));
@@ -1305,6 +1340,9 @@
             return MTB_ERR_INTERNAL;
         case kErrLiveCount:
             set_error("internal error: K5 kept more live matches than a read's segment holds");
+            return MTB_ERR_INTERNAL;
+        case kErrRunIndex:
+            set_error("internal error: K5's group or species-run count of a read differs from the live pack's");
             return MTB_ERR_INTERNAL;
         default:
             set_error("internal error: device error flag " + std::to_string(err));
diff --git a/metabuli_work_amd/csrc/mtb_assign.hip b/metabuli_work_amd/csrc/mtb_assign.hip
--- a/metabuli_work_amd/csrc/mtb_assign.hip
+++ b/metabuli_work_amd/csrc/mtb_assign.hip
@@ -102,6 +102,33 @@
     return SegIn{seg, inOff[r] * (inCS & 0xFFFFu), (uint64_t)(r + 1) << 32};
 }
 
+struct RunCnt {
+    uint32_t* __restrict__ grp;
+    uint32_t* __restrict__ run;
+    __device__ __forceinline__ void put(uint32_t r, uint32_t ng, uint32_t ns) const {
+        if (grp) {
+            grp[r] = ng;
+            run[r] = ns;
+        }
+    }
+};
+
+template <int E>
+__device__ __forceinline__ void count_runs(const uint64_t (&sf)[E], const bool (&on)[E], int lane, uint32_t& ng,
+                                           uint32_t& ns) {
+    uint64_t prevLast = 0;
+    ng = ns = 0;
+#pragma unroll
+    for (int sl = 0; sl < E; sl++) {
+        uint64_t pv = __shfl_up(sf[sl], 1, 64);
+        if (lane == 0) pv = prevLast;
+        prevLast = __shfl(sf[sl], 63, 64);
+        const bool first = sl == 0 && lane == 0;
+        ng += (uint32_t)__popcll(__ballot(on[sl] && (first || pv != sf[sl])));
+        ns += (uint32_t)__popcll(__ballot(on[sl] && (first || (pv >> 3) != (sf[sl] >> 3))));
+    }
+}
+
 template <typename K>
 __device__ __forceinline__ uint32_t lds_insert(K* tab, uint32_t tn, K key) {
     uint32_t i = (uint32_t)(((uint64_t)key * 0x9E3779B97F4A7C15ull) >> 40) & (tn - 1);
@@ -115,7 +142,7 @@
 template <int E2>
 __device__ __forceinline__ void sort_live(mtb_match* __restrict__ out, uint64_t seqBits,
                                           uint64_t base, int nLive, int lane, const uint64_t* cH,
-                                          const uint64_t* cL, const uint32_t* cX) {
+                                          const uint64_t* cL, const uint32_t* cX, uint32_t& ng, uint32_t& ns) {
     uint64_t h[E2], l[E2];
     uint32_t x[E2];
 #pragma unroll
@@ -127,6 +154,14 @@
         x[sl] = v ? cX[e] : 0u;
     }
     wave_bitonic_sort<E2>(h, l, x, lane);
+    uint64_t sf[E2];
+    bool on[E2];
+#pragma unroll
+    for (int sl = 0; sl < E2; sl++) {
+        sf[sl] = h[sl] >> 29;
+        on[sl] = 64 * sl + lane < nLive;
+    }
+    count_runs<E2>(sf, on, lane, ng, ns);
 #pragma unroll
     for (int sl = 0; sl < E2; sl++) {
         const int e = 64 * sl + lane;
@@ -171,7 +206,7 @@
 
 template <int E, typename In>
 __device__ __forceinline__ void prune_then_sort(const In& in, mtb_match* __restrict__ out, uint64_t base, int n, int lane,
-                                                uint32_t* __restrict__ liveCnt, uint32_t r, uint32_t pm) {
+                                                uint32_t* __restrict__ liveCnt, uint32_t r, uint32_t pm, RunCnt rc) {
     constexpr uint32_t T = 128 * E;
     constexpr uint32_t kLive = 0x80000000u;
     PruneLds<E>& L = prune_lds<E>();
@@ -224,11 +259,15 @@
     }
     __syncthreads();
     const uint64_t seqBits = nLive ? in.full(0).qinfo & (0x1FFFFFFFull << 32) : 0;
-    if (nLive <= 64) sort_live<1>(out, seqBits, base, nLive, lane, cH, cL, cX);
-    else if (E >= 2 && nLive <= 128) sort_live<(E >= 2 ? 2 : 1)>(out, seqBits, base, nLive, lane, cH, cL, cX);
-    else if (E >= 4 && nLive <= 256) sort_live<(E >= 4 ? 4 : 1)>(out, seqBits, base, nLive, lane, cH, cL, cX);
-    else sort_live<E>(out, seqBits, base, nLive, lane, cH, cL, cX);
-    if (lane == 0) liveCnt[r] = (uint32_t)nLive;
+    uint32_t ng = 0, ns = 0;
+    if (nLive <= 64) sort_live<1>(out, seqBits, base, nLive, lane, cH, cL, cX, ng, ns);
+    else if (E >= 2 && nLive <= 128) sort_live<(E >= 2 ? 2 : 1)>(out, seqBits, base, nLive, lane, cH, cL, cX, ng, ns);
+    else if (E >= 4 && nLive <= 256) sort_live<(E >= 4 ? 4 : 1)>(out, seqBits, base, nLive, lane, cH, cL, cX, ng, ns);
+    else sort_live<E>(out, seqBits, base, nLive, lane, cH, cL, cX, ng, ns);
+    if (lane == 0) {
+        liveCnt[r] = (uint32_t)nLive;
+        rc.put(r, ng, ns);
+    }
 }
 
 template <int E, typename K>
@@ -312,7 +351,7 @@
 
 template <int E, typename In>
 __device__ __forceinline__ void prune_rank_sort(const In& in, mtb_match* __restrict__ out, uint64_t base, int n, int lane,
-                                                uint32_t* __restrict__ liveCnt, uint32_t r, uint32_t pm) {
+                                                uint32_t* __restrict__ liveCnt, uint32_t r, uint32_t pm, RunCnt rc) {
     constexpr uint32_t T = 128 * E;
     constexpr uint32_t kLive = 0x80000000u;
     RankLds<E>& L = rank_lds<E>();
@@ -402,8 +441,14 @@
     lds_sort_keys_n<E, uint64_t>(L.c.key, nLive, lane);
     __syncthreads();
     const uint64_t seqBits = nLive ? in.full(0).qinfo & (0x1FFFFFFFull << 32) : 0;
-    for (int e = lane; e < nLive; e += 64) {
-        const uint64_t k = L.c.key[e];
+    uint32_t ng = 0, ns = 0;
+    for (int e0 = 0; e0 < nLive; e0 += 64) {
+        const int e = e0 + lane;
+        const bool on = e < nLive;
+        const uint64_t k = on ? L.c.key[e] : 0, pk = on && e ? L.c.key[e - 1] : 0;
+        ng += (uint32_t)__popcll(__ballot(on && (e == 0 || (pk >> frameAt) != (k >> frameAt))));
+        ns += (uint32_t)__popcll(__ballot(on && (e == 0 || (pk >> (frameAt + 3)) != (k >> (frameAt + 3)))));
+        if (!on) continue;
         const uint32_t p = (uint32_t)(k & 511u);
         const uint64_t pre = k >> 9, lo = L.c.lo[p];
         int at = e;
@@ -419,12 +464,16 @@
         m.pad = 0;
         out[base + at] = m;
     }
-    if (lane == 0) liveCnt[r] = (uint32_t)nLive;
+    if (lane == 0) {
+        liveCnt[r] = (uint32_t)nLive;
+        rc.put(r, ng, ns);
+    }
 }
 
 template <int E, typename In>
 __device__ __forceinline__ void sort_then_prune(const In& in, mtb_match* __restrict__ out, uint64_t base, int n,
-                                                int lane, uint32_t* __restrict__ liveCnt, uint32_t r, uint32_t pm) {
+                                                int lane, uint32_t* __restrict__ liveCnt, uint32_t r, uint32_t pm,
+                                                RunCnt rc) {
     uint64_t h[E], l[E];
     uint32_t x[E];
 #pragma unroll
@@ -444,6 +493,7 @@
     uint8_t* runLive = run_live_lds<E>();
     const uint64_t lt = (1ull << lane) - 1;
     const int far = lane + (int)pm - 1;
+    constexpr uint32_t kRidMask = 0x3FFFFFFFu;
     uint32_t rid[E];
     bool pair[E];
     uint32_t runs = 0;
@@ -460,21 +510,24 @@
         pair[sl] = e + (int)pm - 1 < n && (far < 64 ? a : b) == sf;
         const bool start = e < n && (e == 0 || (pv >> 3) != (sf >> 3));
         const uint64_t m = __ballot(start);
-        rid[sl] = runs + (uint32_t)__popcll(m & lt) + (uint32_t)start - 1u;
+        rid[sl] = (runs + (uint32_t)__popcll(m & lt) + (uint32_t)start - 1u) | (uint32_t)start << 31 |
+                  (uint32_t)(e < n && (e == 0 || pv != sf)) << 30;
         runs += (uint32_t)__popcll(m);
         runLive[64 * sl + lane] = 0;
     }
     __syncthreads();
 #pragma unroll
     for (int sl = 0; sl < E; sl++)
-        if (pair[sl]) runLive[rid[sl]] = 1;
-    __syncthreads();
-    uint32_t kept = 0;
+        if (pair[sl]) runLive[rid[sl] & kRidMask] = 1;
+    __syncthreads();
+    uint32_t kept = 0, ng = 0, ns = 0;
 #pragma unroll
     for (int sl = 0; sl < E; sl++) {
         const int e = 64 * sl + lane;
-        const bool live = e < n && runLive[rid[sl]];
+        const bool live = e < n && runLive[rid[sl] & kRidMask];
         const uint64_t m = __ballot(live);
+        ng += (uint32_t)__popcll(__ballot(live && (rid[sl] >> 30 & 1u)));
+        ns += (uint32_t)__popcll(__ballot(live && rid[sl] >> 31));
         if (live) {
             mtb_match o;
             o.qinfo = ((h[sl] >> 29) & 7ull) << 61 | seqBits | (uint32_t)(h[sl] & 0x1FFFFFFFu);
@@ -488,26 +541,29 @@
         }
         kept += (uint32_t)__popcll(m);
     }
-    if (lane == 0) liveCnt[r] = kept;
+    if (lane == 0) {
+        liveCnt[r] = kept;
+        rc.put(r, ng, ns);
+    }
 }
 
 template <int E, typename In, int kMode = 2>
 __device__ __forceinline__ void segsort_regs(const In& in, mtb_match* __restrict__ out, uint64_t base, int n, int lane,
-                                             uint32_t* __restrict__ liveCnt, uint32_t r, uint32_t pm) {
+                                             uint32_t* __restrict__ liveCnt, uint32_t r, uint32_t pm, RunCnt rc) {
     if constexpr (E >= 2 && kMode == 2) {
         if (liveCnt) {
-            prune_rank_sort<E>(in, out, base, n, lane, liveCnt, r, pm);
+            prune_rank_sort<E>(in, out, base, n, lane, liveCnt, r, pm, rc);
             return;
         }
         if constexpr (E > 2) return;
     } else if constexpr (E >= 2 && kMode == 1) {
         if (liveCnt && pm <= 64) {
-            sort_then_prune<E>(in, out, base, n, lane, liveCnt, r, pm);
+            sort_then_prune<E>(in, out, base, n, lane, liveCnt, r, pm, rc);
             return;
         }
     } else if constexpr (E >= 2 && kMode == 0) {
         if (liveCnt) {
-            prune_then_sort<E>(in, out, base, n, lane, liveCnt, r, pm);
+            prune_then_sort<E>(in, out, base, n, lane, liveCnt, r, pm, rc);
             return;
         }
         if constexpr (E > 2) return;
@@ -557,28 +613,41 @@
         if (pair[sl]) runLive[rid[sl]] = 1;
     __syncthreads();
     uint32_t kept = 0;
+    uint64_t sf[E];
+    bool on[E];
 #pragma unroll
     for (int sl = 0; sl < E; sl++) {
         const int e = 64 * sl + lane;
         const bool live = e < n && runLive[rid[sl]];
         const uint64_t m = __ballot(live);
+        sf[sl] = h[sl] >> 29;
+        on[sl] = live;
         if (live) out[base + kept + (uint32_t)__popcll(m & lt)] = in.full(x[sl]);
         kept += (uint32_t)__popcll(m);
     }
-    if (lane == 0) liveCnt[r] = kept;
+    uint32_t ng, ns;
+    count_runs<E>(sf, on, lane, ng, ns);
+    if (lane == 0) {
+        liveCnt[r] = kept;
+        rc.put(r, ng, ns);
+    }
     }
 }
 
 template <typename In>
 __device__ __forceinline__ void segsort_small_run(const In& in, mtb_match* __restrict__ out, uint64_t base, int n,
-                                                  int lane, uint32_t* __restrict__ liveCnt, uint32_t r, uint32_t pm) {
+                                                  int lane, uint32_t* __restrict__ liveCnt, uint32_t r, uint32_t pm,
+                                                  RunCnt rc) {
     if (n <= 1 || (liveCnt && n < (int)pm)) {
         if (lane == 0 && n == 1 && !liveCnt) out[base] = in.full(0);
-        if (lane == 0 && liveCnt) liveCnt[r] = 0;
+        if (lane == 0 && liveCnt) {
+            liveCnt[r] = 0;
+            rc.put(r, 0, 0);
+        }
         return;
     }
-    if (n <= 64) segsort_regs<1>(in, out, base, n, lane, liveCnt, r, pm);
-    else segsort_regs<2>(in, out, base, n, lane, liveCnt, r, pm);
+    if (n <= 64) segsort_regs<1>(in, out, base, n, lane, liveCnt, r, pm, rc);
+    else segsort_regs<2>(in, out, base, n, lane, liveCnt, r, pm, rc);
 }
 
 __global__ void __launch_bounds__(64) k_segsort_small(const mtb_match* __restrict__ in, const uint64_t* __restrict__ mOff,
@@ -586,15 +655,17 @@
                                                       const uint64_t* __restrict__ inOff, uint32_t inC,
                                                       uint32_t nReads, mtb_match* __restrict__ out,
                                                       uint32_t* __restrict__ liveCnt, uint32_t pm,
-                                                      const uint32_t* __restrict__ segLen) {
+                                                      const uint32_t* __restrict__ segLen,
+                                                      uint32_t* __restrict__ grpCnt) {
     const uint32_t r = blockIdx.x;
     if (r >= nReads) return;
     const uint64_t base = mOff[r];
     const long nl = seg_len(mOff, segLen, r);
     if (nl < 0 || nl > 128) return;
     const int n = (int)nl;
-    if (sparse_read(seg, inOff, inC, r, n)) segsort_small_run(sparse_in(seg, inOff, inC, r), out, base, n, threadIdx.x, liveCnt, r, pm);
-    else segsort_small_run(MatchIn{in, base}, out, base, n, threadIdx.x, liveCnt, r, pm);
+    const RunCnt rc{grpCnt, grpCnt ? grpCnt + nReads + 1 : nullptr};
+    if (sparse_read(seg, inOff, inC, r, n)) segsort_small_run(sparse_in(seg, inOff, inC, r), out, base, n, threadIdx.x, liveCnt, r, pm, rc);
+    else segsort_small_run(MatchIn{in, base}, out, base, n, threadIdx.x, liveCnt, r, pm, rc);
 }
 
 template <int E, int kMode>
@@ -604,18 +675,20 @@
                                                      uint32_t nReads, mtb_match* __restrict__ out,
                                                      uint32_t* __restrict__ liveCnt, uint32_t pm,
                                                      const uint32_t* __restrict__ segLen,
-                                                     const uint32_t* __restrict__ list) {
+                                                     const uint32_t* __restrict__ list,
+                                                     uint32_t* __restrict__ grpCnt) {
     const uint32_t r = list ? list[blockIdx.x] : blockIdx.x;
     if (r >= nReads) return;
     const uint64_t base = mOff[r];
     const long nl = seg_len(mOff, segLen, r);
     if (nl <= 32 * E || nl > 64 * E) return;
     const int n = (int)nl;
+    const RunCnt rc{grpCnt, grpCnt ? grpCnt + nReads + 1 : nullptr};
     if (sparse_read(seg, inOff, inC, r, n))
         segsort_regs<E, SegIn, kMode>(sparse_in(seg, inOff, inC, r), out, base, n,
-                                       (int)threadIdx.x, liveCnt, r, pm);
+                                       (int)threadIdx.x, liveCnt, r, pm, rc);
     else
-        segsort_regs<E, MatchIn, kMode>(MatchIn{in, base}, out, base, n, (int)threadIdx.x, liveCnt, r, pm);
+        segsort_regs<E, MatchIn, kMode>(MatchIn{in, base}, out, base, n, (int)threadIdx.x, liveCnt, r, pm, rc);
 }
 
 template <int kThreads, typename Idx>
@@ -1018,7 +1091,8 @@
                                                                  uint64_t* __restrict__ gScratch, int global,
                                                                  uint32_t* __restrict__ liveCnt, long mergeSeg, uint32_t pm,
                                                                  const uint32_t* __restrict__ segLen, int compact,
-                                                                 const uint32_t* __restrict__ list) {
+                                                                 const uint32_t* __restrict__ list,
+                                                                 uint32_t* __restrict__ grpCnt) {
     __shared__ uint64_t sh[kBlockSeg], sl[kBlockSeg];
     __shared__ uint16_t si[kBlockSeg];
     const uint32_t r = list ? list[blockIdx.x] : blockIdx.x;
@@ -1026,7 +1100,10 @@
     const uint64_t base = mOff[r];
     long n = seg_len(mOff, segLen, r);
     if (n < 0) return;
-    if (global && n == 0 && liveCnt && threadIdx.x == 0) liveCnt[r] = 0;
+    if (global && n == 0 && liveCnt && threadIdx.x == 0) {
+        liveCnt[r] = 0;
+        RunCnt{grpCnt, grpCnt ? grpCnt + nReads + 1 : nullptr}.put(r, 0, 0);
+    }
     if (global ? n == 0 : n <= kMidSeg) return;
     __shared__ uint32_t sWave[kLargeThreads / 64 + 1];
     long p2 = 2;
@@ -1433,11 +1510,11 @@
 static hipError_t launch_sorts(const mtb_match* in, const uint64_t* mOff, uint32_t nReads, uint64_t M, mtb_match* out,
                                uint64_t* gScratch, uint32_t maxSeg, uint32_t* liveCnt, long chunk, uint32_t pm,
                                const uint32_t* segLen, hipStream_t s, const SegMatch* seg, const uint64_t* inOff,
-                               uint32_t inC, int mode, uint32_t* lists) {
-    k_segsort_small<<<nReads, 64, 0, s>>>(in, mOff, seg, inOff, inC, nReads, out, liveCnt, pm, segLen);
+                               uint32_t inC, int mode, uint32_t* lists, uint32_t* grpCnt) {
+    k_segsort_small<<<nReads, 64, 0, s>>>(in, mOff, seg, inOff, inC, nReads, out, liveCnt, pm, segLen, grpCnt);
     if (maxSeg <= 128) return hipGetLastError();
     if (!lists) {
-#define MTB_REGS(E, M) k_segsort_regs<E, M><<<nReads, 64, 0, s>>>(in, mOff, seg, inOff, inC, nReads, out, liveCnt, pm, segLen, nullptr)
+#define MTB_REGS(E, M) k_segsort_regs<E, M><<<nReads, 64, 0, s>>>(in, mOff, seg, inOff, inC, nReads, out, liveCnt, pm, segLen, nullptr, grpCnt)
         if (!liveCnt) mode = 3;
         if (maxSeg > 128) {
             if (mode == 1) MTB_REGS(4, 1);
@@ -1457,7 +1534,7 @@
                                                          inC, mode == 2 ? 1 : mode == 4 ? 2 : 0, nullptr);
         if (maxSeg > kMidSeg)
             k_segsort_large<<<nReads, kLargeThreads, 0, s>>>(in, mOff, nReads, M, out, gScratch, 0, liveCnt, chunk, pm,
-                                                             segLen, mode == 2 ? 1 : mode == 4 ? 2 : 0, nullptr);
+                                                             segLen, mode == 2 ? 1 : mode == 4 ? 2 : 0, nullptr, nullptr);
         MTB_HIP_RET(hipGetLastError());
         if (maxSeg > chunk) return launch_merge_path(in, mOff, nReads, M, out, gScratch, liveCnt, chunk, pm, segLen, s);
         return hipSuccess;
@@ -1476,7 +1553,7 @@
     const uint32_t* listMid = lists + 2 * (size_t)nReads;
     const uint32_t* listLarge = lists + 3 * (size_t)nReads;
 #define MTB_REGS(E, M, N, L) \
-    k_segsort_regs<E, M><<<N, 64, 0, s>>>(in, mOff, seg, inOff, inC, nReads, out, liveCnt, pm, segLen, L)
+    k_segsort_regs<E, M><<<N, 64, 0, s>>>(in, mOff, seg, inOff, inC, nReads, out, liveCnt, pm, segLen, L, grpCnt)
     if (!liveCnt) mode = 3;
     if (e == hipSuccess && cnt[0]) {
         if (mode == 1) MTB_REGS(4, 1, cnt[0], list4);
@@ -1496,7 +1573,7 @@
                                                      mode == 2 ? 1 : mode == 4 ? 2 : 0, listMid);
     if (e == hipSuccess && cnt[3])
         k_segsort_large<<<cnt[3], kLargeThreads, 0, s>>>(in, mOff, nReads, M, out, gScratch, 0, liveCnt, chunk, pm,
-                                                         segLen, mode == 2 ? 1 : mode == 4 ? 2 : 0, listLarge);
+                                                         segLen, mode == 2 ? 1 : mode == 4 ? 2 : 0, listLarge, nullptr);
     if (e == hipSuccess) e = hipGetLastError();
     MTB_HIP_RET(e);
     if (maxSeg > chunk) return launch_merge_path(in, mOff, nReads, M, out, gScratch, liveCnt, chunk, pm, segLen, s);
@@ -1506,23 +1583,26 @@
 hipError_t launch_segsort(const mtb_match* in, const uint64_t* mOff, uint32_t nReads, uint64_t M, mtb_match* out,
                           uint64_t* gScratch, uint32_t maxSeg, bool global, uint32_t* liveCnt, uint32_t mergeSeg,
                           uint32_t pm, hipStream_t s, const SegMatch* seg, const uint64_t* inOff, uint32_t inC,
-                          uint32_t* segLen, uint32_t* maxTmp, int after, uint32_t* lists) {
+                          uint32_t* segLen, uint32_t* maxTmp, int after, uint32_t* lists, uint32_t* grpCnt,
+                          bool* counted) {
     pm = max(pm, 2u);
+    const bool counts = liveCnt && grpCnt && !global && maxSeg <= (uint32_t)kSmallSeg && (after != 1 || pm <= 64);
+    if (counted) *counted = counts;
     if (nReads == 0) return hipSuccess;
     const bool thin = liveCnt && segLen;
     if (seg && (global || (maxSeg > kSegSortSparse && !thin))) return hipErrorInvalidValue;
     const long chunk = std::max<long>(kSmallSeg, std::min<long>(mergeSeg ? mergeSeg : kBlockSeg, kBlockSeg));
     if (global) {
         k_segsort_large<<<nReads, kLargeThreads, 0, s>>>(in, mOff, nReads, M, out, gScratch, 1, liveCnt, chunk, pm,
-                                                         nullptr, 0, nullptr);
+                                                         nullptr, 0, nullptr, grpCnt);
         return hipGetLastError();
     }
     const long thinAbove = std::min<long>(chunk, kMidSeg);
     if (!liveCnt || maxSeg <= (uint32_t)thinAbove || !segLen)
         return launch_sorts(in, mOff, nReads, M, out, gScratch, maxSeg, liveCnt, chunk, pm, nullptr, s, seg, inOff, inC, after,
-                            lists);
+                            lists, counts ? grpCnt : nullptr);
     MTB_HIP_RET(launch_sorts(in, mOff, nReads, M, out, gScratch, (uint32_t)thinAbove, liveCnt, chunk, pm, nullptr, s,
-                             seg, inOff, inC, after, lists));
+                             seg, inOff, inC, after, lists, nullptr));
     mtb_match* io = const_cast<mtb_match*>(in);
     k_thin_big<<<nReads, kLargeThreads, 0, s>>>(io, out, mOff, nReads, thinAbove, pm, segLen, seg, inOff, inC);
     MTB_HIP_RET(hipMemsetAsync(maxTmp, 0, sizeof(uint32_t), s));
@@ -1532,30 +1612,47 @@
     MTB_HIP_RET(hipStreamSynchronize(s));
     if (maxSurv == 0) return hipSuccess;
     return launch_sorts(in, mOff, nReads, M, out, gScratch, maxSurv, liveCnt, chunk, pm, segLen, s, nullptr, nullptr, 0, after,
-                        lists);
-}
-
-template <bool kCopy>
+                        lists, nullptr);
+}
+
+template <bool kCopy, bool kIndex>
 __global__ void __launch_bounds__(256) k_run_flags(const mtb_match* __restrict__ in, const uint64_t* __restrict__ mOff,
                                                    const uint64_t* __restrict__ liveOff, uint32_t nReads,
                                                    mtb_match* __restrict__ out, uint8_t* __restrict__ flags,
                                                    uint32_t* __restrict__ grpCnt, uint32_t* __restrict__ runCnt,
-                                                   int* __restrict__ err) {
+                                                   int* __restrict__ err, const uint64_t* __restrict__ grpOff,
+                                                   const uint64_t* __restrict__ runOff, uint64_t* __restrict__ gStart,
+                                                   uint64_t* __restrict__ sStart, uint64_t* __restrict__ runGroup) {
     const uint32_t r = blockIdx.x * 4 + threadIdx.x / 64;
     const uint32_t lane = threadIdx.x & 63;
     if (r >= nReads) return;
     const uint64_t lo = liveOff[r];
     const uint64_t live = liveOff[r + 1] - lo;
+    uint64_t g0 = 0, s0 = 0;
+    uint32_t gN = 0, sN = 0;
+    if (kIndex) {
+        g0 = grpOff[r];
+        s0 = runOff[r];
+        gN = (uint32_t)(grpOff[r + 1] - g0);
+        sN = (uint32_t)(runOff[r + 1] - s0);
+    }
+    if (kIndex && r == nReads - 1 && lane == 0) {
+        gStart[grpOff[nReads]] = liveOff[nReads];
+        sStart[runOff[nReads]] = liveOff[nReads];
+    }
     if (kCopy && (live > mOff[r + 1] - mOff[r] || liveOff[r + 1] > mOff[nReads])) {
         if (lane == 0) {
             atomicExch(err, kErrLiveCount);
-            grpCnt[r] = 0;
-            runCnt[r] = 0;
+            if (!kIndex) {
+                grpCnt[r] = 0;
+                runCnt[r] = 0;
+            }
         }
         return;
     }
     const mtb_match* src = in + (kCopy ? mOff[r] : lo);
     uint32_t ng = 0, ns = 0;
+    const unsigned long long below = (1ull << lane) - 1;
     for (uint64_t e0 = 0; e0 < live; e0 += 64) {
         const uint64_t e = e0 + lane;
         const bool on = e < live;
@@ -1571,12 +1668,26 @@
         const bool newG = on && (newSp || pfr != fr);
         if (on) {
             if (kCopy) out[lo + e] = m;
-            flags[lo + e] = (uint8_t)((uint32_t)newG | (uint32_t)newSp << 1);
-        }
-        ng += (uint32_t)__popcll(__ballot(newG));
-        ns += (uint32_t)__popcll(__ballot(newSp));
-    }
-    if (lane == 0) {
+            if (!kIndex) flags[lo + e] = (uint8_t)((uint32_t)newG | (uint32_t)newSp << 1);
+        }
+        const unsigned long long mg = __ballot(newG), ms = __ballot(newSp);
+        if (kIndex) {
+            const uint32_t g = ng + (uint32_t)__popcll(mg & below);
+            if (newG && g < gN) gStart[g0 + g] = lo + e;
+            if (newSp) {
+                const uint32_t sr = ns + (uint32_t)__popcll(ms & below);
+                if (sr < sN && g < gN) {
+                    sStart[s0 + sr] = lo + e;
+                    runGroup[s0 + sr] = g0 + g;
+                }
+            }
+        }
+        ng += (uint32_t)__popcll(mg);
+        ns += (uint32_t)__popcll(ms);
+    }
+    if (kIndex) {
+        if (lane == 0 && (ng != gN || ns != sN)) atomicExch(err, kErrRunIndex);
+    } else if (lane == 0) {
         grpCnt[r] = ng;
         runCnt[r] = ns;
     }
@@ -1585,8 +1696,20 @@
 void launch_run_flags(const mtb_match* in, const uint64_t* mOff, const uint64_t* liveOff, uint32_t nReads,
                       mtb_match* out, uint8_t* flags, uint32_t* grpCnt, uint32_t* runCnt, int* err, hipStream_t s) {
     if (!nReads) return;
-    if (out) k_run_flags<true><<<(nReads + 3) / 4, 256, 0, s>>>(in, mOff, liveOff, nReads, out, flags, grpCnt, runCnt, err);
-    else k_run_flags<false><<<(nReads + 3) / 4, 256, 0, s>>>(in, mOff, liveOff, nReads, out, flags, grpCnt, runCnt, err);
+    if (out)
+        k_run_flags<true, false><<<(nReads + 3) / 4, 256, 0, s>>>(in, mOff, liveOff, nReads, out, flags, grpCnt, runCnt, err,
+                                                                   nullptr, nullptr, nullptr, nullptr, nullptr);
+    else
+        k_run_flags<false, false><<<(nReads + 3) / 4, 256, 0, s>>>(in, mOff, liveOff, nReads, out, flags, grpCnt, runCnt,
+                                                                    err, nullptr, nullptr, nullptr, nullptr, nullptr);
+}
+
+void launch_pack_index(const mtb_match* in, const uint64_t* mOff, const uint64_t* liveOff, uint32_t nReads,
+                       mtb_match* out, const uint64_t* grpOff, const uint64_t* runOff, uint64_t* gStart,
+                       uint64_t* sStart, uint64_t* runGroup, int* err, hipStream_t s) {
+    if (!nReads) return;
+    k_run_flags<true, true><<<(nReads + 3) / 4, 256, 0, s>>>(in, mOff, liveOff, nReads, out, nullptr, nullptr, nullptr, err,
+                                                              grpOff, runOff, gStart, sStart, runGroup);
 }
 
 __global__ void __launch_bounds__(256) k_max_seg(const uint64_t* __restrict__ off, uint32_t n, uint32_t* __restrict__ out) {
@@ -2914,22 +3037,31 @@
     return inB ? s.ordVB : s.ordVA;
 }
 
-void launch_assign(const mtb_match* matches, const uint64_t* mOff, const uint32_t* qlen, uint32_t nReads, uint64_t nM, const AssignArgs& a, const TaxDevice& t, const AssignScratch& s,
-                   mtb_taxcnt* tcPool, mtb_result* results, unsigned long long* devStats, uint64_t* hostStats,
-                   hipStream_t st) {
+int launch_assign(const mtb_match* matches, const uint64_t* mOff, const uint32_t* qlen, uint32_t nReads, uint64_t nM, const AssignArgs& a, const TaxDevice& t, const AssignScratch& s,
+                  mtb_taxcnt* tcPool, mtb_result* results, unsigned long long* devStats, uint64_t* hostStats,
+                  hipStream_t st) {
     for (int i = 0; i < 4; i++) hostStats[i] = 0;
-    if (nReads == 0) return;
+    if (nReads == 0) return 0;
     AssignCfg cfg{a.kmerFormat, a.dnaShift, a.maxCodonShift, a.denominator, a.minConsCnt, a.minConsCntEuk,
                   a.accessionLevel, a.minScore, a.minSpScore, a.tieRatio, a.generic, a.emulateAll, a.em};
     TaxView tv{t.nodeOf, t.nodeTax, t.parent, t.depth, t.flags, t.spParent, t.maxTax};
-    exclusive_scan_u32(s.grpCnt, nReads, s.grpOff, s.scanTmp, st);
-    exclusive_scan_u32(s.runCnt, nReads, s.runOff, s.scanTmp, st);
+    if (!s.indexBuilt) {
+        exclusive_scan_u32(s.grpCnt, nReads, s.grpOff, s.scanTmp, st);
+        exclusive_scan_u32(s.runCnt, nReads, s.runOff, s.scanTmp, st);
+    }
     if (nM) {
-        launch_run_starts(s.runFlag, mOff, s.grpOff, s.runOff, nReads, s.gStart, s.sStart, s.runGroup, st);
-        uint64_t cnt[2] = {0, 0};
-        hipMemcpyAsync(&cnt[0], s.grpOff + nReads, sizeof(uint64_t), hipMemcpyDeviceToHost, st);
-        hipMemcpyAsync(&cnt[1], s.runOff + nReads, sizeof(uint64_t), hipMemcpyDeviceToHost, st);
+        if (!s.indexBuilt)
+            launch_run_starts(s.runFlag, mOff, s.grpOff, s.runOff, nReads, s.gStart, s.sStart, s.runGroup, st);
+        uint64_t cnt[2] = {s.idxGroups, s.idxRuns};
+        int err = 0;
+        if (s.indexBuilt) {
+            hipMemcpyAsync(&err, s.err, sizeof(int), hipMemcpyDeviceToHost, st);
+        } else {
+            hipMemcpyAsync(&cnt[0], s.grpOff + nReads, sizeof(uint64_t), hipMemcpyDeviceToHost, st);
+            hipMemcpyAsync(&cnt[1], s.runOff + nReads, sizeof(uint64_t), hipMemcpyDeviceToHost, st);
+        }
         hipStreamSynchronize(st);
+        if (err == kErrRunIndex || err == kErrLiveCount) return err;
         hostStats[0] = cnt[0];
         hostStats[2] = cnt[1];
         if (cnt[0]) {
@@ -3004,6 +3136,7 @@
                                                              s.runGroup, s.gStart, s.spScore, s.spKeep, cfg, tv,
                                                              (Clade*)s.clade, s.cladePerMatch, tcPool, results);
     }
+    return 0;
 }
 
 uint64_t path_bytes() { return sizeof(Path); }
diff --git a/metabuli_work_amd/csrc/mtb_launch.h b/metabuli_work_amd/csrc/mtb_launch.h
--- a/metabuli_work_amd/csrc/mtb_launch.h
+++ b/metabuli_work_amd/csrc/mtb_launch.h
@@ -14,6 +14,7 @@
 constexpr int kErrProbeCount = 4;
 constexpr int kErrRunOutsideDb = 5;
 constexpr int kErrLiveCount = 6;
+constexpr int kErrRunIndex = 7;
 
 struct ReadMeta {
     int32_t len1, len2, ql1, ql2, w1, w2;
@@ -56,6 +57,9 @@
     const uint8_t* runFlag;
     const uint32_t *grpCnt, *runCnt;
     uint64_t *grpOff, *runOff;
+    bool indexBuilt;
+    const int* err;
+    uint64_t idxGroups, idxRuns;
     float* spScore;
     uint64_t* waveList;
     uint32_t* waveCount;
@@ -264,7 +268,8 @@
                           uint32_t pruneMin, hipStream_t s, const SegMatch* seg = nullptr,
                           const uint64_t* inOff = nullptr, uint32_t inC = 0 ,
                           uint32_t* segLen = nullptr,
-                          uint32_t* maxTmp = nullptr, int pruneAfter = 0, uint32_t* lists = nullptr);
+                          uint32_t* maxTmp = nullptr, int pruneAfter = 0, uint32_t* lists = nullptr,
+                          uint32_t* grpCnt = nullptr, bool* counted = nullptr);
 inline uint32_t prune_min_matches(int minConsCnt, int minConsCntEuk, int maxCodonShift) {
     const int d = minConsCnt < minConsCntEuk ? minConsCnt : minConsCntEuk;
     const int sh = maxCodonShift > 0 ? maxCodonShift : 1;
@@ -273,15 +278,18 @@
 }
 void launch_run_flags(const mtb_match* in, const uint64_t* mOff, const uint64_t* liveOff, uint32_t nReads,
                       mtb_match* out, uint8_t* flags, uint32_t* grpCnt, uint32_t* runCnt, int* err, hipStream_t s);
+void launch_pack_index(const mtb_match* in, const uint64_t* mOff, const uint64_t* liveOff, uint32_t nReads,
+                       mtb_match* out, const uint64_t* grpOff, const uint64_t* runOff, uint64_t* gStart,
+                       uint64_t* sStart, uint64_t* runGroup, int* err, hipStream_t s);
 void launch_max_u32(const uint32_t* x, uint32_t n, uint32_t* out, hipStream_t s);
 void launch_max_seg(const uint64_t* off, uint32_t n, uint32_t* out, hipStream_t s);
 constexpr uint32_t kSegSortLds = 8192;
 constexpr uint32_t kSegSortRegs = 512;
 constexpr uint32_t kSegSortSparse = 2048;
 constexpr uint64_t kMaxBatchMatches = 0xFFFFFFFFull;
-void launch_assign(const mtb_match* matches, const uint64_t* mOff, const uint32_t* qlen, uint32_t nReads, uint64_t nM, const AssignArgs& a, const TaxDevice& t, const AssignScratch& s,
-                   mtb_taxcnt* tcPool, mtb_result* results, unsigned long long* devStats, uint64_t* hostStats,
-                   hipStream_t st);
+int launch_assign(const mtb_match* matches, const uint64_t* mOff, const uint32_t* qlen, uint32_t nReads, uint64_t nM, const AssignArgs& a, const TaxDevice& t, const AssignScratch& s,
+                  mtb_taxcnt* tcPool, mtb_result* results, unsigned long long* devStats, uint64_t* hostStats,
+                  hipStream_t st);
 void launch_regroup_chunks(const mtb_match* src, const uint32_t* cnt, uint32_t nChunks, uint32_t n, uint32_t* tot,
                            uint64_t* srcOff, uint64_t* mOff, void* scanTmp, mtb_match* dst, hipStream_t s);
 void launch_taxcnt_len(const mtb_result* results, uint32_t nReads, uint32_t* len, hipStream_t s);
```

Result: no change. 34.85 million (median of 6 runs) (+0.6%).
